# KirillHit/snn_for_object_detection

Hardware: AMD Instinct MI355X
Metric: event-frames/sec (BxT) SODa-3M GEN1 304x240 fwd+bwd (higher is better)
Workload: dtype f32 (16-bit split products)

## Files before the change

### include/snn_hip.h

```cpp
#ifndef SNN_HIP_H
#define SNN_HIP_H

#include <stddef.h>
#include <stdint.h>

#ifdef __cplusplus
extern "C" {
#endif

#define SNN_ABI_VERSION 11

enum {
    SNN_NEURON_NONE = 0,
    SNN_NEURON_LIF = 1,
    SNN_NEURON_LI = 2,
    SNN_NEURON_LI_TANH = 3,
    SNN_NEURON_SLI = 4,
    SNN_NEURON_SYNAPSE = 5
};

enum { SNN_PREC_FP32 = 0, SNN_PREC_BF16X3 = 1, SNN_PREC_BF16X6 = 3, SNN_PREC_FP16X3 = 4, SNN_PREC_BF16X1 = 5,
       SNN_PREC_BF16S = 6 };

enum { SNN_SCAN_WIDE_ADDRESSING = 1,
       SNN_SCAN_LAST_STEP_ONLY = 2,
       SNN_SCAN_BF16_STORAGE = 4,
       SNN_SCAN_SPIKES_FROM_VDEC = 8,
       SNN_SCAN_SUMS_FROM_STATE = 16,
       SNN_SCAN_STATE_LOOKBACK = 32   };

enum { SNN_POOL_AVG = 0, SNN_POOL_MAX = 1, SNN_POOL_SUM = 2 };

enum { SNN_ACT_RELU = 0, SNN_ACT_SILU = 1, SNN_ACT_TANH = 2 };

typedef struct snn_neuron_params {
    float c_mem;
    float c_syn;
    float v_leak;
    float v_th;
    float v_reset;
    float alpha;
    float v_st;
    float tau_sec;
    float tau_dis;
    float dt;
    float sigma;
} snn_neuron_params;

int snn_abi_version(void);
const char* snn_last_error(void);

int snn_nchw_to_nhwc(const float* src, float* dst, int64_t N, int C, int H, int W, void* stream);
int snn_nhwc_to_nchw(const float* src, float* dst, int64_t N, int C, int H, int W, void* stream);
int snn_weight_transpose(const float* w, float* wt, int Cout, int KH, int KW, int Cin, void* stream);
int snn_weight_transpose_batched(const float* flat_w, float* flat_wt, const int64_t* table, int n_layers, void* stream);
int snn_weight_presplit(const float* w, void* out, int64_t n, int precision, void* stream);

int snn_conv2d_wgrad_bn_supported(int64_t N, int H, int W, int Cin, int Ho, int Wo, int Cout, int KH, int KW, int stride,
                                  int pad);
int snn_conv2d_wgrad_bn(const float* x, int64_t ldx, const float* gx, int64_t ldgx, const float* y, int64_t ldy,
                        const float* coef, int T, int frames_per_step, float* dw, int64_t N, int H, int W, int Cin, int Ho,
                        int Wo, int Cout, int KH, int KW, int stride, int pad, int accumulate, float* workspace, int splitk,
                        void* stream);
int snn_conv3x3_s2_dgrad_supported(int64_t N, int H, int W, int Cin, int Ho, int Wo, int Cout);
int snn_conv3x3_s2_dgrad(const float* dy, int64_t lddy, const void* wt_image, float* dx, int64_t lddx, int64_t N, int H, int W,
                         int Cin, int Ho, int Wo, int Cout, const float* addend, int64_t ld_addend, const float* addend2,
                         int64_t ld_addend2, int precision , void* stream);
int snn_conv3x3_halo_bn_supported(int64_t N, int H, int W, int Cin, int Cout, int frames_per_step);
int snn_conv3x3_halo_bn(const float* gx, const float* y, const float* coef, int frames_per_step, float* dy_out,
                        const void* wt_image, float* dx, int64_t lddx, int64_t N, int H, int W, int Cin, int Cout,
                        const float* addend, int64_t ld_addend, const float* addend2, int64_t ld_addend2, void* stream);
int snn_conv3x3_halo_supported(int64_t N, int H, int W, int Cin, int Cout);
int64_t snn_conv3x3_halo_bn_chunks(int frames_per_step, int H, int W);
size_t snn_weight_frag_image_bytes(int O, int I);
int snn_weight_frag_image_batched(const float* flat_src, void* flat_dst, const int64_t* table, int n, int max_threads,
                                  int flip, int precision, void* stream);
int snn_conv3x3_halo(const float* x, int64_t ldx, const void* w_image, float* y, int64_t ldy, int64_t N, int H, int W,
                     int Cin, int Cout, const float* addend, int64_t ld_addend, const float* addend2, int64_t ld_addend2,
                     double* bn_partial, int frames_per_step, int* bn_layout, int precision, void* stream);
size_t snn_conv2d_fwd_bn_partial_size(int64_t N, int frames_per_step, int Ho, int Wo, int Cout);
int snn_conv2d_fwd(const float* x, int64_t ldx, const float* w, const void* w_split, float* y, int64_t ldy,
                   int64_t N, int H, int W, int Cin, int Ho, int Wo, int Cout,
                   int KH, int KW, int stride, int pad, const float* addend, int64_t ld_addend,
                   double* bn_partial, int frames_per_step, int* bn_layout, int precision, void* stream);
int snn_conv2d_dgrad(const float* dy, int64_t lddy, const float* wt, const void* wt_split, float* dx, int64_t lddx,
                     int64_t N, int H, int W, int Cin, int Ho, int Wo, int Cout,
                     int KH, int KW, int stride, int pad, const float* addend, int64_t ld_addend,
                     const float* addend2, int64_t ld_addend2, int precision, void* stream);
int snn_conv2d_wgrad(const float* x, int64_t ldx, const float* dy, int64_t lddy, float* dw,
                     int64_t N, int H, int W, int Cin, int Ho, int Wo, int Cout,
                     int KH, int KW, int stride, int pad, int accumulate,
                     float* workspace, int splitk, int precision, void* stream);
int snn_conv2d_wgrad_splitk(int64_t N, int H, int W, int Cin, int Ho, int Wo, int Cout, int KH, int KW,
                            int stride, int pad, int precision);
int snn_conv2d_wgrad_kernel(int64_t N, int H, int W, int Cin, int Ho, int Wo, int Cout, int KH, int KW, int stride, int pad,
                            int precision);
int snn_conv1x1_spikes_supported(int64_t N, int H, int W, int Cin, int Cout, int64_t ld, int fwd_precision,
                                 int bwd_precision);
int snn_conv1x1_spikes_fwd(const float* vdec, int64_t ld, float v_th, const float* w, float* y, int64_t ldy, int64_t N, int H,
                           int W, int Cin, int Cout, void* stream);
int snn_conv1x1_spikes_wgrad(const float* vdec, int64_t ld, float v_th, const float* dy, int64_t lddy, float* dw, int64_t N,
                             int H, int W, int Cin, int Cout, int accumulate, float* workspace, int splitk, void* stream);

int snn_conv2d_spikes_supported(int64_t N, int H, int W, int Cin, int Ho, int Wo, int Cout, int KH, int KW, int stride,
                                int pad, int64_t ld, int fwd_precision, int bwd_precision);
int snn_conv2d_spikes_fwd(const float* vdec, int64_t ld, float v_th, const float* w, float* y, int64_t ldy, int64_t N, int H,
                          int W, int Cin, int Ho, int Wo, int Cout, int KH, int KW, int stride, int pad, double* bn_partial,
                          int frames_per_step, int* bn_layout, void* stream);
int snn_conv2d_spikes_wgrad(const float* vdec, int64_t ld, float v_th, const float* dy, int64_t lddy, float* dw, int64_t N,
                            int H, int W, int Cin, int Ho, int Wo, int Cout, int KH, int KW, int stride, int pad,
                            int accumulate, float* workspace, int splitk, void* stream);
int snn_conv3x3_halo_spikes(const float* vdec, int64_t ld, float v_th, const void* w_image, float* y, int64_t ldy, int64_t N,
                            int H, int W, int Cin, int Cout, double* bn_partial, int frames_per_step, int* bn_layout,
                            void* stream);

size_t snn_bn_stats_partial_size(int T, int64_t M, int C);
int snn_bn_stats(const float* y, int64_t ldy, int T, int64_t M, int C, double* partial, void* stream);
int snn_bn_stats_finalize(const double* partial, int chunks, int rows_per_chunk, int T, int64_t M, int C,
                          const float* gamma, const float* bias, float eps, float momentum,
                          float* running_mean, float* running_var, int use_running,
                          float* mean, float* invstd, float* alpha, float* beta, void* stream);

int snn_bn_stats_reduce(const double* partial, int chunks, int rows_per_chunk, int T, int64_t M, int C, double* sums,
                        void* stream);
int snn_bn_stats_from_sums(const double* sums, int T, int64_t M_total, int C,
                           const float* gamma, const float* bias, float eps, float momentum,
                           float* running_mean, float* running_var,
                           float* mean, float* invstd, float* alpha, float* beta,
                           double* var_scratch, void* stream);

int snn_affine_neuron_fwd(int neuron, const float* y, int64_t ldy,
                          const float* alpha, const float* beta,
                          const float* v0, const float* i0,
                          float* out, int64_t ldo, const float* addend, int64_t ld_addend,
                          float* vT, float* iT, float* vdec,
                          int T, int64_t M, int C, const snn_neuron_params* p, int flags, void* stream);

size_t snn_affine_neuron_bwd_sums_size(int T, int64_t M, int C);
int snn_affine_neuron_bwd_sums_from_state(int neuron, int T, int64_t M, int C, int64_t ldg, const snn_neuron_params* p,
                                          int flags);
int snn_affine_neuron_bwd(int neuron, const float* g_out, int64_t ldg, const float* state,
                          const float* y, int64_t ldy, const float* g_vT, const float* g_iT,
                          const float* alpha, const float* beta, int apply_scale,
                          float* gx, float* g_v0, float* g_i0, double* sums,
                          int T, int64_t M, int C, const snn_neuron_params* p, int flags, void* stream);

int snn_lif_ckpt_interval(void);
int snn_lif_fwd_ckpt(const float* y, int64_t ldy, const float* alpha, const float* beta,
                     const float* v0, const float* i0, float* out, int64_t ldo,
                     const float* addend, int64_t ld_addend, float* vT, float* iT, float* ckpt,
                     int T, int64_t M, int C, const snn_neuron_params* p, void* stream);
int snn_lif_bwd_ckpt(const float* g_out, int64_t ldg, const float* ckpt, const float* y, int64_t ldy,
                     const float* g_vT, const float* g_iT, const float* alpha, const float* beta, int apply_scale,
                     float* gx, float* g_v0, float* g_i0, double* sums,
                     int T, int64_t M, int C, const snn_neuron_params* p, void* stream);

int snn_bn_bwd_finalize(double* sums, int T, int64_t M, int C,
                        const float* gamma, const float* mean, const float* invstd,
                        float* coefA, float* coefB, float* coefC,
                        float* dgamma, float* dbias, int accumulate, void* stream);
int snn_bn_bwd_finalize_from_state(double* sums, int T, int64_t M, int C,
                                   const float* gamma, const float* bias, const float* mean, const float* invstd,
                                   const float* gx, const float* y, int64_t ldy,
                                   float* coefA, float* coefB, float* coefC,
                                   float* dgamma, float* dbias, int accumulate, void* stream);
int snn_bn_bwd_reduce(const double* sums, int T, int64_t M, int C, double* raw, void* stream);
int snn_bn_bwd_reduce_from_state(const double* sums, int T, int64_t M, int C, const float* gamma, const float* bias,
                                 const float* mean, const float* invstd, const float* gx, const float* y, int64_t ldy,
                                 double* raw, void* stream);
int snn_bn_bwd_coef(const double* raw, const double* raw_local, double* param_sums, int T, int64_t M_total, int C,
                    const float* gamma, const float* mean, const float* invstd,
                    float* coefA, float* coefB, float* coefC,
                    float* dgamma, float* dbias, int accumulate, void* stream);
int snn_bn_bwd_apply(const float* gx, const float* y, int64_t ldy,
                     const float* coefA, const float* coefB, const float* coefC,
                     float* dy, int64_t lddy, int T, int64_t M, int C, int accumulate, void* stream);
int snn_bn_bwd_apply_bf16(const float* gx, const float* y, int64_t ldy, const float* coefA, const float* coefB,
                          const float* coefC, float* dy, int64_t lddy, int T, int64_t M, int C, int accumulate, void* stream);
int snn_bn_stats_bf16(const float* y, int64_t ldy, int T, int64_t M, int C, double* partial, void* stream);

int snn_copy_channels(const float* src, int64_t lds, float* dst, int64_t ldd, int64_t M, int C, void* stream);
int snn_add_channels(const float* src, int64_t lds, float* dst, int64_t ldd, int64_t M, int C, void* stream);
int snn_add(const float* a, int64_t lda, const float* b, int64_t ldb, float* dst, int64_t ldd,
            int64_t M, int C, void* stream);
int snn_copy_channels_bf16(const float* src, int64_t lds, float* dst, int64_t ldd, int64_t M, int C, void* stream);
int snn_add_bf16(const float* a, int64_t lda, const float* b, int64_t ldb, float* dst, int64_t ldd, int64_t M, int C,
                 void* stream);
int snn_convert_bf16(const void* src, void* dst, int64_t n, int to_bf16, void* stream);
int snn_act_fwd(int act, const float* x, float* y, int64_t n, void* stream);
int snn_act_bwd(int act, const float* x, const float* y, const float* gy, float* gx, int64_t n, void* stream);

int snn_small_gemm(const float* A, int64_t lda, int transA, const float* B, int64_t ldb, int transB, float* C,
                  int64_t ldc, int M, int N, int K, int accumulate, float* Ct, int64_t ldct, void* stream);
int snn_small_gemm_batched(const float* base_a, const float* base_b, float* base_c, float* base_ct, const int64_t* table,
                           int n, int max_tiles, void* stream);

int snn_lstm_cell_fwd(const float* gates, const float* c_prev, float* h, float* c, int64_t M, int C, void* stream);
int snn_lstm_cell_bwd(const float* gates, const float* c_prev, const float* c, const float* gh, const float* gc,
                      float* g_gates, float* g_c_prev, int64_t M, int C, void* stream);

int snn_pool_fwd(int kind, const float* x, float* y, int64_t N, int H, int W, int C,
                 int Ho, int Wo, int k, int stride, void* stream);
int snn_pool_bwd(int kind, const float* x, const float* gy, float* gx, int64_t N, int H, int W, int C,
                 int Ho, int Wo, int k, int stride, void* stream);
int snn_upsample_fwd(const float* x, float* y, int64_t N, int H, int W, int C, int scale, void* stream);
int snn_upsample_bwd(const float* gy, float* gx, int64_t N, int H, int W, int C, int scale, void* stream);

int snn_adamax_step(float* param, const float* grad, float* exp_avg, float* exp_inf,
                    int64_t n, float lr, float beta1, float beta2, float eps, int step,
                    float grad_scale, void* stream);

int snn_events_to_frames(const int32_t* t_bin, const int32_t* x, const int32_t* y, const int32_t* p,
                         int64_t n_events, float* frames, int T, int H, int W, void* stream);

int snn_detect_decode(const float* cls_prob, const float* offsets, const float* anchors, int A, int K,
                      float* conf, int* cls, float* boxes, void* stream);
int snn_nms_sorted(const float* boxes, const int* order, const int* seg, int num_classes, float iou_threshold,
                   int* kept, int* nkept, unsigned char* kept_flag, int* kept_rank, void* stream);

size_t snn_roi_workspace_size(int B, int A, int N);
int snn_roi_assign(const float* anchors, const float* labels, int B, int A, int N, float iou_threshold,
                   void* workspace, float* bbox_offset, float* bbox_mask, int64_t* class_labels, void* stream);
size_t snn_det_loss_workspace_size(int64_t rows);
int snn_det_loss_fwd(const float* cls_logits, const float* bbox_preds, const float* bbox_offset, const float* bbox_mask,
                     const int64_t* class_labels, int64_t rows, int K, float loss_ratio, void* workspace, double* stats,
                     float* loss, void* stream);
int snn_det_loss_bwd(const float* cls_logits, const float* bbox_preds, const float* bbox_offset, const float* bbox_mask,
                     const int64_t* class_labels, int64_t rows, int K, float loss_ratio, const double* stats,
                     const float* g_loss, float* g_logits, float* g_bbox, void* stream);

#ifdef __cplusplus
}
#endif
#endif
```

### snn_for_object_detection_amd/_hip.py

```python

import ctypes
import os
from ctypes import POINTER, Structure, c_char_p, c_double, c_float, c_int, c_int32, c_int64, c_size_t, c_void_p

_HERE = os.path.dirname(os.path.abspath(__file__))
LIB_PATH = os.environ.get("SNN_HIP_LIB") or os.path.join(_HERE, "libsnn_hip.so")

NEURON_NONE, NEURON_LIF, NEURON_LI, NEURON_LI_TANH, NEURON_SLI, NEURON_SYNAPSE = 0, 1, 2, 3, 4, 5
POOL_AVG, POOL_MAX, POOL_SUM = 0, 1, 2
ACT_RELU, ACT_SILU, ACT_TANH = 0, 1, 2
ABI_VERSION = 11
PREC_FP32, PREC_BF16X3, PREC_BF16X6, PREC_FP16X3, PREC_BF16X1, PREC_BF16S = 0, 1, 3, 4, 5, 6
SCAN_WIDE_ADDRESSING, SCAN_LAST_STEP_ONLY, SCAN_BF16_STORAGE, SCAN_SPIKES_FROM_VDEC, SCAN_SUMS_FROM_STATE = 1, 2, 4, 8, 16
SCAN_STATE_LOOKBACK = 32


class NeuronParams(Structure):
    _fields_ = [("c_mem", c_float), ("c_syn", c_float), ("v_leak", c_float), ("v_th", c_float),
                ("v_reset", c_float), ("alpha", c_float), ("v_st", c_float), ("tau_sec", c_float),
                ("tau_dis", c_float), ("dt", c_float), ("sigma", c_float)]


_P, _I, _L, _F = c_void_p, c_int, c_int64, c_float

SIGNATURES = {
    "snn_abi_version": (c_int, []),
    "snn_last_error": (c_char_p, []),
    "snn_nchw_to_nhwc": (c_int, [_P, _P, _L, _I, _I, _I, _P]),
    "snn_nhwc_to_nchw": (c_int, [_P, _P, _L, _I, _I, _I, _P]),
    "snn_weight_transpose": (c_int, [_P, _P, _I, _I, _I, _I, _P]),
    "snn_weight_transpose_batched": (c_int, [_P, _P, _P, _I, _P]),
    "snn_detect_decode": (c_int, [_P, _P, _P, _I, _I, _P, _P, _P, _P]),
    "snn_nms_sorted": (c_int, [_P, _P, _P, _I, _F, _P, _P, _P, _P, _P]),
    "snn_conv2d_fwd": (c_int, [_P, _L, _P, _P, _P, _L, _L, _I, _I, _I, _I, _I, _I, _I, _I, _I, _I, _P, _L, _P, _I, _P, _I,
                               _P]),
    "snn_weight_presplit": (c_int, [_P, _P, _L, _I, _P]),
    "snn_conv2d_fwd_bn_partial_size": (c_size_t, [_L, _I, _I, _I, _I]),
    "snn_conv2d_wgrad_bn_supported": (c_int, [_L, _I, _I, _I, _I, _I, _I, _I, _I, _I, _I]),
    "snn_conv2d_wgrad_bn": (c_int, [_P, _L, _P, _L, _P, _L, _P, _I, _I, _P, _L, _I, _I, _I, _I, _I, _I, _I, _I, _I, _I, _I,
                                    _P, _I, _P]),
    "snn_conv3x3_s2_dgrad_supported": (c_int, [_L, _I, _I, _I, _I, _I, _I]),
    "snn_conv3x3_s2_dgrad": (c_int, [_P, _L, _P, _P, _L, _L, _I, _I, _I, _I, _I, _I, _P, _L, _P, _L, _I, _P]),
    "snn_conv3x3_halo_bn_supported": (c_int, [_L, _I, _I, _I, _I, _I]),
    "snn_conv3x3_halo_bn": (c_int, [_P, _P, _P, _I, _P, _P, _P, _L, _L, _I, _I, _I, _I, _P, _L, _P, _L, _P]),
    "snn_conv3x3_halo_supported": (c_int, [_L, _I, _I, _I, _I]),
    "snn_conv3x3_halo_bn_chunks": (c_int64, [_I, _I, _I]),
    "snn_weight_frag_image_bytes": (c_size_t, [_I, _I]),
    "snn_weight_frag_image_batched": (c_int, [_P, _P, _P, _I, _I, _I, _I, _P]),
    "snn_conv3x3_halo": (c_int, [_P, _L, _P, _P, _L, _L, _I, _I, _I, _I, _P, _L, _P, _L, _P, _I, _P, _I, _P]),
    "snn_conv2d_dgrad": (c_int, [_P, _L, _P, _P, _P, _L, _L, _I, _I, _I, _I, _I, _I, _I, _I, _I, _I, _P, _L, _P, _L,
                                 _I, _P]),
    "snn_conv2d_wgrad": (c_int, [_P, _L, _P, _L, _P, _L, _I, _I, _I, _I, _I, _I, _I, _I, _I, _I, _I, _P, _I, _I,
                                 _P]),
    "snn_conv2d_wgrad_splitk": (c_int, [_L, _I, _I, _I, _I, _I, _I, _I, _I, _I, _I, _I]),
    "snn_conv2d_wgrad_kernel": (c_int, [_L, _I, _I, _I, _I, _I, _I, _I, _I, _I, _I, _I]),
    "snn_conv1x1_spikes_supported": (c_int, [_L, _I, _I, _I, _I, _L, _I, _I]),
    "snn_conv1x1_spikes_fwd": (c_int, [_P, _L, _F, _P, _P, _L, _L, _I, _I, _I, _I, _P]),
    "snn_conv1x1_spikes_wgrad": (c_int, [_P, _L, _F, _P, _L, _P, _L, _I, _I, _I, _I, _I, _P, _I, _P]),
    "snn_conv2d_spikes_supported": (c_int, [_L, _I, _I, _I, _I, _I, _I, _I, _I, _I, _I, _L, _I, _I]),
    "snn_conv2d_spikes_fwd": (c_int, [_P, _L, _F, _P, _P, _L, _L, _I, _I, _I, _I, _I, _I, _I, _I, _I, _I, _P, _I, _P, _P]),
    "snn_conv2d_spikes_wgrad": (c_int, [_P, _L, _F, _P, _L, _P, _L, _I, _I, _I, _I, _I, _I, _I, _I, _I, _I, _I, _P, _I, _P]),
    "snn_conv3x3_halo_spikes": (c_int, [_P, _L, _F, _P, _P, _L, _L, _I, _I, _I, _I, _P, _I, _P, _P]),
    "snn_bn_stats_partial_size": (c_size_t, [_I, _L, _I]),
    "snn_bn_stats": (c_int, [_P, _L, _I, _L, _I, _P, _P]),
    "snn_bn_stats_finalize": (c_int, [_P, _I, _I, _I, _L, _I, _P, _P, _F, _F, _P, _P, _I, _P, _P, _P, _P, _P]),
    "snn_bn_stats_reduce": (c_int, [_P, _I, _I, _I, _L, _I, _P, _P]),
    "snn_bn_stats_from_sums": (c_int, [_P, _I, _L, _I, _P, _P, _F, _F, _P, _P, _P, _P, _P, _P, _P, _P]),
    "snn_bn_bwd_reduce": (c_int, [_P, _I, _L, _I, _P, _P]),
    "snn_bn_bwd_coef": (c_int, [_P, _P, _P, _I, _L, _I, _P, _P, _P, _P, _P, _P, _P, _P, _I, _P]),
    "snn_affine_neuron_fwd": (c_int, [_I, _P, _L, _P, _P, _P, _P, _P, _L, _P, _L, _P, _P, _P, _I, _L, _I,
                                      POINTER(NeuronParams), _I, _P]),
    "snn_lif_ckpt_interval": (c_int, []),
    "snn_lif_fwd_ckpt": (c_int, [_P, _L, _P, _P, _P, _P, _P, _L, _P, _L, _P, _P, _P, _I, _L, _I,
                                 POINTER(NeuronParams), _P]),
    "snn_lif_bwd_ckpt": (c_int, [_P, _L, _P, _P, _L, _P, _P, _P, _P, _I, _P, _P, _P, _P, _I, _L, _I,
                                 POINTER(NeuronParams), _P]),
    "snn_affine_neuron_bwd_sums_size": (c_size_t, [_I, _L, _I]),
    "snn_affine_neuron_bwd": (c_int, [_I, _P, _L, _P, _P, _L, _P, _P, _P, _P, _I, _P, _P, _P, _P, _I, _L, _I,
                                      POINTER(NeuronParams), _I, _P]),
    "snn_bn_bwd_finalize": (c_int, [_P, _I, _L, _I, _P, _P, _P, _P, _P, _P, _P, _P, _I, _P]),
    "snn_bn_bwd_finalize_from_state": (c_int, [_P, _I, _L, _I, _P, _P, _P, _P, _P, _P, _L, _P, _P, _P, _P, _P, _I, _P]),
    "snn_bn_bwd_reduce_from_state": (c_int, [_P, _I, _L, _I, _P, _P, _P, _P, _P, _P, _L, _P, _P]),
    "snn_affine_neuron_bwd_sums_from_state": (c_int, [_I, _I, _L, _I, _L, POINTER(NeuronParams), _I]),
    "snn_bn_bwd_apply": (c_int, [_P, _P, _L, _P, _P, _P, _P, _L, _I, _L, _I, _I, _P]),
    "snn_bn_bwd_apply_bf16": (c_int, [_P, _P, _L, _P, _P, _P, _P, _L, _I, _L, _I, _I, _P]),
    "snn_bn_stats_bf16": (c_int, [_P, _L, _I, _L, _I, _P, _P]),
    "snn_copy_channels": (c_int, [_P, _L, _P, _L, _L, _I, _P]),
    "snn_add_channels": (c_int, [_P, _L, _P, _L, _L, _I, _P]),
    "snn_add": (c_int, [_P, _L, _P, _L, _P, _L, _L, _I, _P]),
    "snn_roi_workspace_size": (c_size_t, [_I, _I, _I]),
    "snn_roi_assign": (c_int, [_P, _P, _I, _I, _I, _F, _P, _P, _P, _P, _P]),
    "snn_det_loss_workspace_size": (c_size_t, [_L]),
    "snn_det_loss_fwd": (c_int, [_P, _P, _P, _P, _P, _L, _I, _F, _P, _P, _P, _P]),
    "snn_det_loss_bwd": (c_int, [_P, _P, _P, _P, _P, _L, _I, _F, _P, _P, _P, _P, _P]),
    "snn_small_gemm": (c_int, [_P, _L, _I, _P, _L, _I, _P, _L, _I, _I, _I, _I, _P, _L, _P]),
    "snn_small_gemm_batched": (c_int, [_P, _P, _P, _P, _P, _I, _I, _P]),
    "snn_copy_channels_bf16": (c_int, [_P, _L, _P, _L, _L, _I, _P]),
    "snn_add_bf16": (c_int, [_P, _L, _P, _L, _P, _L, _L, _I, _P]),
    "snn_convert_bf16": (c_int, [_P, _P, _L, _I, _P]),
    "snn_act_fwd": (c_int, [_I, _P, _P, _L, _P]),
    "snn_act_bwd": (c_int, [_I, _P, _P, _P, _P, _L, _P]),
    "snn_lstm_cell_fwd": (c_int, [_P, _P, _P, _P, _L, _I, _P]),
    "snn_lstm_cell_bwd": (c_int, [_P, _P, _P, _P, _P, _P, _P, _L, _I, _P]),
    "snn_pool_fwd": (c_int, [_I, _P, _P, _L, _I, _I, _I, _I, _I, _I, _I, _P]),
    "snn_pool_bwd": (c_int, [_I, _P, _P, _P, _L, _I, _I, _I, _I, _I, _I, _I, _P]),
    "snn_upsample_fwd": (c_int, [_P, _P, _L, _I, _I, _I, _I, _P]),
    "snn_upsample_bwd": (c_int, [_P, _P, _L, _I, _I, _I, _I, _P]),
    "snn_adamax_step": (c_int, [_P, _P, _P, _P, _L, _F, _F, _F, _F, _I, _F, _P]),
    "snn_events_to_frames": (c_int, [_P, _P, _P, _P, _L, _P, _I, _I, _I, _P]),
}

_lib = None


def load():
    global _lib
    if _lib is not None:
        return _lib
    if not os.path.exists(LIB_PATH):
        raise RuntimeError(
            f"{LIB_PATH} not found: the gfx950 HIP extension has not been built "
            "(run `python -m snn_for_object_detection_amd._build`); there is no CPU / eager fallback")
    if not os.environ.get("SNN_HIP_LIB"):
        from . import _build
        if not _build.library_is_current():
            raise RuntimeError(
                f"{LIB_PATH} was not built from the kernel sources as they are now (csrc/*.hip, include/snn_hip.h "
                "changed, or the build stamp is missing): run `python -m snn_for_object_detection_amd._build`")
    lib = ctypes.CDLL(LIB_PATH)
    for name, (res, args) in SIGNATURES.items():
        fn = getattr(lib, name)
        fn.restype, fn.argtypes = res, args
    if lib.snn_abi_version() != ABI_VERSION:
        raise RuntimeError(f"libsnn_hip.so ABI {lib.snn_abi_version()} != binding {ABI_VERSION}: rebuild")
    _lib = lib
    return lib


PROFILER = None


def call(name: str, *args) -> None:
    lib = load()
    if PROFILER is not None:
        token = PROFILER.before(name, args)
        rc = getattr(lib, name)(*args)
        PROFILER.after(token)
    else:
        rc = getattr(lib, name)(*args)
    if rc != 0:
        msg = lib.snn_last_error()
        raise RuntimeError(f"{name} failed (rc={rc}): {msg.decode() if msg else '?'}")


def query(name: str, *args):
    return getattr(load(), name)(*args)
```

### snn_for_object_detection_amd/csrc/conv_halo.hip

```cpp
#include <stdlib.h>
#include <type_traits>
#include "snn_common.h"

namespace {

constexpr int kThreads = 256;
constexpr int HBM_ = 128;
constexpr int HCELLS = 288;
constexpr int HPIECE = HCELLS * 64;
constexpr int NPASS = HCELLS / 32;
static_assert(NPASS == 9, "one halo staging pass per tap");

typedef __bf16 bf16x8 __attribute__((ext_vector_type(8)));
typedef __bf16 bf16x2 __attribute__((ext_vector_type(2)));
typedef _Float16 f16x8 __attribute__((ext_vector_type(8)));
typedef _Float16 f16x2 __attribute__((ext_vector_type(2)));
typedef float f32x2 __attribute__((ext_vector_type(2)));
typedef unsigned u32x2 __attribute__((ext_vector_type(2)));
typedef unsigned u32x4 __attribute__((ext_vector_type(4)));

constexpr float kF16WeightScale = 256.0f;
constexpr float kF16ActScale = 16.0f;
constexpr float kF16Unscale = 1.0f / (kF16WeightScale * kF16ActScale);

struct HaloGeom {
    int64_t ldx, ldy, ld_add, ld_add2;
    int N, H, W, Cin, Cout;
    int PW, PH;
    int G;
    int group_cells;
    int tiles_per_group, tiles, tiles_per_xcd, ntiles_n;
    unsigned magic_pw, magic_ph;
    int out_vec;
    double* bn_partial;
    int OH, OW;
    int bn_T, bn_tc, bn_fps;
    int tiles_x, tiles_img;
    float x_th;
};

__device__ __forceinline__ unsigned udiv_small(unsigned n, unsigned magic) { return __umulhi(n, magic); }

template <bool F16>
__device__ __forceinline__ void split4(const f32x4& v, u32x2& hi, u32x2& lo) {
#pragma unroll
    for (int e = 0; e < 4; e += 2) {
        if constexpr (F16) {
            const float a = v[e] * kF16ActScale, b = v[e + 1] * kF16ActScale;
            const f16x2 ph = __builtin_convertvector(f32x2{a, b}, f16x2);
            const f16x2 pl = __builtin_convertvector(f32x2{a - (float)ph[0], b - (float)ph[1]}, f16x2);
            hi[e >> 1] = __builtin_bit_cast(unsigned, ph);
            lo[e >> 1] = __builtin_bit_cast(unsigned, pl);
        } else {
            f32x2 rest = {v[e], v[e + 1]};
            const bf16x2 ph = __builtin_convertvector(rest, bf16x2);
            const unsigned bits = __builtin_bit_cast(unsigned, ph);
            rest[0] -= __builtin_bit_cast(float, bits << 16);
            rest[1] -= __builtin_bit_cast(float, bits & 0xffff0000u);
            const bf16x2 pl = __builtin_convertvector(rest, bf16x2);
            hi[e >> 1] = bits;
            lo[e >> 1] = __builtin_bit_cast(unsigned, pl);
        }
    }
}

__device__ __forceinline__ double partner8(double v) {
    const u32x2 u = __builtin_bit_cast(u32x2, v);
    const u32x2 o = {(unsigned)__builtin_amdgcn_update_dpp(0, (int)u[0], 0x128, 0xf, 0xf, false),
                     (unsigned)__builtin_amdgcn_update_dpp(0, (int)u[1], 0x128, 0xf, 0xf, false)};
    return __builtin_bit_cast(double, o);
}
__device__ __forceinline__ double partner16(double v) {
    const u32x2 u = __builtin_bit_cast(u32x2, v);
    const u32x2 o = {__builtin_amdgcn_permlane16_swap(u[0], u[0], false, false)[0],
                     __builtin_amdgcn_permlane16_swap(u[1], u[1], false, false)[0]};
    return __builtin_bit_cast(double, o);
}
__device__ __forceinline__ double partner32(double v) {
    const u32x2 u = __builtin_bit_cast(u32x2, v);
    const u32x2 o = {__builtin_amdgcn_permlane32_swap(u[0], u[0], false, false)[0],
                     __builtin_amdgcn_permlane32_swap(u[1], u[1], false, false)[0]};
    return __builtin_bit_cast(double, o);
}

__device__ __forceinline__ int cell_slot_off(int cell, int slot) { return cell * 64 + ((slot ^ ((cell >> 2) & 3)) << 4); }

constexpr int BN_NT = 3;
constexpr int BN_CMAX = 128;

constexpr int RTH = 4, RTW = 32, RPITCH = RTW + 2, RCELLS = (RTH + 2) * RPITCH;

template <int CO, bool F16, int ABL = 0, bool BNAP = false, bool RECT = false, bool SBF = false, bool XSP = false>
__global__ __launch_bounds__(kThreads, 2) void k_conv_halo3(const float* __restrict__ x,
                                                           const unsigned char* __restrict__ wimg,
                                                           float* __restrict__ y, HaloGeom g,
                                                           const float* __restrict__ addend,
                                                           const float* __restrict__ addend2,
                                                           const float* __restrict__ bn_y = nullptr,
                                                           const float* __restrict__ bn_coef = nullptr,
                                                           float* __restrict__ dy_out = nullptr) {
    constexpr int WM = CO == 32 ? 4 : 2, WN = 4 / WM, TM = CO == 32 ? 1 : 2, TN = CO == 32 ? 1 : CO / 64;
    static_assert(CO == 32 || CO == 64 || CO == 128, "channel tile");
    static_assert(!BNAP || CO >= 64, "the BatchNorm-apply variant covers the 64 / 128-channel tiles");
    constexpr int BTILE = (CO / 32) * 4096;
    constexpr int NDMA = (CO / 32) * 4 / 4;
    constexpr int ES = SBF ? 2 : 4;
    static_assert(!SBF || (!F16 && !BNAP && ABL == 0), "bf16 storage: bf16 MFMA, plain variant");
    static_assert(!XSP || (F16 && !BNAP && !SBF && ABL == 0), "spikes from potentials: the forward arithmetic, plain variant");
    constexpr int CF_BYTES = BNAP ? 3 * BN_NT * BN_CMAX * 4 : 0;
    constexpr int HC = RECT ? (RCELLS + 31) / 32 * 32 : HCELLS;
    constexpr int HP = HC * 64;
    constexpr int RED_BYTES = (F16 || SBF) ? 4 * (CO == 128 ? 64 : 32) * 16 : 0;
    __shared__ __attribute__((aligned(16))) unsigned char smem[2 * HP + 2 * BTILE + CF_BYTES + RED_BYTES];
    unsigned char* Aimg = smem;
    unsigned char* Bimg = smem + 2 * HP;
    [[maybe_unused]] float* Cf = reinterpret_cast<float*>(smem + 2 * HP + 2 * BTILE);

    const int tid = threadIdx.x, lane = tid & 63;
    const int wave = __builtin_amdgcn_readfirstlane(tid >> 6);
    const int wm = wave / WN, wn = wave % WN;
    const int r = lane & 31, h = lane >> 5;

    const int bq = blockIdx.x >> 3;
    const int tile = (blockIdx.x & 7) * g.tiles_per_xcd + bq / g.ntiles_n;
    if (tile >= g.tiles) return;
    const int n0c = (bq % g.ntiles_n) * CO;
    int grp, kt, c0 = 0, x0 = 0, y0 = 0, n0, nb;
    [[maybe_unused]] int ty = 0, tx = 0;
    if constexpr (RECT) {
        n0 = tile / g.tiles_img;
        const int rem = tile - n0 * g.tiles_img;
        ty = rem / g.tiles_x;
        tx = rem - ty * g.tiles_x;
        grp = n0 / g.G;
        kt = (n0 - grp * g.G) * g.tiles_img + rem;
        nb = n0;
    } else {
        grp = tile / g.tiles_per_group;
        kt = tile - grp * g.tiles_per_group;
        c0 = kt * HBM_;
        const int R0g = c0 / g.PW;
        x0 = c0 - R0g * g.PW;
        const int ng = R0g / g.PH;
        y0 = R0g - ng * g.PH;
        n0 = grp * g.G + ng;
        nb = n0 > 0 ? n0 - 1 : 0;
    }
    const int pitch = RECT ? RPITCH : g.PW;

    const int quad = tid & 7;
    const int64_t ipix = (int64_t)g.H * g.W;
    const int64_t xbytes = ((((int64_t)g.N - nb) * ipix - 1) * g.ldx + g.Cin) * ES;
    __amdgpu_buffer_rsrc_t rs_x = __builtin_amdgcn_make_buffer_rsrc(
        reinterpret_cast<char*>(const_cast<float*>(x)) + (int64_t)nb * ipix * g.ldx * ES, 0,
        xbytes > 0x7fffffffLL ? 0x7fffffff : (int)xbytes, 0x00020000);
    [[maybe_unused]] __amdgpu_buffer_rsrc_t rs_y = rs_x, rs_dy = rs_x;
    [[maybe_unused]] const int t_lo = BNAP ? nb / g.bn_fps : 0;
    [[maybe_unused]] int cofs[NPASS];
    [[maybe_unused]] unsigned imask = 0;
    [[maybe_unused]] unsigned vmask = 0;
    if constexpr (BNAP) {
        rs_y = __builtin_amdgcn_make_buffer_rsrc(const_cast<float*>(bn_y + (int64_t)nb * ipix * g.ldx), 0,
                                                 xbytes > 0x7fffffffLL ? 0x7fffffff : (int)xbytes, 0x00020000);
        rs_dy = __builtin_amdgcn_make_buffer_rsrc(dy_out + (int64_t)nb * ipix * g.ldx, 0,
                                                  xbytes > 0x7fffffffLL ? 0x7fffffff : (int)xbytes, 0x00020000);
        for (int idx = tid; idx < 3 * BN_NT * g.Cin; idx += kThreads) {
            const int pl = idx / (BN_NT * g.Cin), rem = idx - pl * BN_NT * g.Cin;
            const int k = rem / g.Cin, c = rem - k * g.Cin;
            const int t = t_lo + k < g.bn_T ? t_lo + k : g.bn_T - 1;
            Cf[idx] = bn_coef[(int64_t)pl * g.bn_tc + (int64_t)t * g.Cin + c];
        }
    }
    unsigned voff[NPASS];
    int awr[NPASS];
#pragma unroll
    for (int p = 0; p < NPASS; ++p) {
        const int cell = p * 32 + (tid >> 3);
        int xx, yy, n;
        bool ok;
        if constexpr (RECT) {
            const int rr = cell / RPITCH, cc = cell - rr * RPITCH;
            yy = ty * RTH - 1 + rr;
            xx = tx * RTW - 1 + cc;
            n = n0;
            ok = cell < RCELLS && yy >= 0 && yy < g.H && xx >= 0 && xx < g.W;
        } else {
            const unsigned u = (unsigned)(x0 + cell + g.PW - 1);
            const unsigned dR = udiv_small(u, g.magic_pw);
            xx = (int)(u - dR * g.PW);
            const unsigned v = (unsigned)(y0 + (int)dR + g.PH - 2);
            const unsigned dn = udiv_small(v, g.magic_ph);
            yy = (int)(v - dn * g.PH);
            n = n0 - 1 + (int)dn;
            ok = n >= 0 && n < g.N && xx < g.W && yy < g.H;
        }
        const int64_t pix = (int64_t)(n - nb) * ipix + (int64_t)yy * g.W + xx;
        voff[p] = ok ? (unsigned)((pix * g.ldx + quad * 4) * ES) : 0x80000000u;
        awr[p] = cell_slot_off(cell, quad >> 1) + (quad & 1) * 8;
        if constexpr (BNAP) {
            int ts = ok ? n / g.bn_fps - t_lo : 0;
            ts = ts < BN_NT ? ts : BN_NT - 1;
            cofs[p] = ts * g.Cin + quad * 4;
            bool mine;
            if constexpr (RECT) {
                const int rr = cell / RPITCH, cc = cell - rr * RPITCH;
                mine = rr >= 1 && rr <= RTH && cc >= 1 && cc <= RTW;
            } else {
                const int m = cell - (g.PW + 1);
                mine = m >= 0 && m < HBM_ && m < g.group_cells - c0;
            }
            imask |= (ok && mine) ? 1u << p : 0u;
            vmask |= ok ? 1u << p : 0u;
        }
    }

    int cellbase[TM];
#pragma unroll
    for (int i = 0; i < TM; ++i)
        cellbase[i] = RECT ? (wm * TM + i + 1) * RPITCH + 1 + r : g.PW + 1 + (wm * TM + i) * 32 + r;
    const int nchunks = g.Cin >> 5;
    const int co_tiles = g.Cout >> 5;
    const unsigned char* wsrc = wimg + (int64_t)(n0c >> 5) * 4096 + lane * 16;
    const unsigned lds_b = (unsigned)(size_t)(__attribute__((address_space(3))) unsigned char*)Bimg;
    auto dma_b = [&](int kk, int buf) {
        if constexpr (SBF)
            if (wave & 1) return;
        const int chunk = kk / 9, tap = kk - chunk * 9;
        const unsigned char* src = wsrc + ((int64_t)(tap * nchunks + chunk) * co_tiles) * 4096 + wave * 1024;
        const unsigned dst = lds_b + buf * BTILE + wave * 1024;
#pragma unroll
        for (int q = 0; q < NDMA; ++q) {
            unsigned keep;
            asm volatile("s_mov_b32 %0, m0\n\ts_mov_b32 m0, %2\n\ts_nop 0\n\tglobal_load_lds_dwordx4 %1, off\n\ts_mov_b32 m0, %0"
                         : "=&s"(keep)
                         : "v"(src + q * 4096), "s"(__builtin_amdgcn_readfirstlane(dst + q * 4096))
                         : "memory");
        }
    };

    using PReg = typename std::conditional<SBF, u32x2, f32x4>::type;
    PReg pf[NPASS];
    auto store_halo = [&]() {
#pragma unroll
        for (int p = 0; p < NPASS; ++p) {
            if constexpr (RECT)
                if (p * 32 >= HC) continue;
            if constexpr (SBF) {
                *reinterpret_cast<u32x2*>(Aimg + awr[p]) = pf[p];
            } else if constexpr (XSP) {
                const u32x2 hi = {(pf[p][0] > g.x_th ? 0x4C00u : 0u) | (pf[p][1] > g.x_th ? 0x4C000000u : 0u),
                                  (pf[p][2] > g.x_th ? 0x4C00u : 0u) | (pf[p][3] > g.x_th ? 0x4C000000u : 0u)};
                *reinterpret_cast<u32x2*>(Aimg + awr[p]) = hi;
            } else {
                u32x2 hi, lo;
                split4<F16>(pf[p], hi, lo);
                *reinterpret_cast<u32x2*>(Aimg + awr[p]) = hi;
                *reinterpret_cast<u32x2*>(Aimg + HP + awr[p]) = lo;
            }
        }
    };
    auto load_pass = [&](int off) -> PReg {
        if constexpr (SBF) return __builtin_bit_cast(u32x2, __builtin_amdgcn_raw_buffer_load_b64(rs_x, off, 0, 0));
        else return __builtin_bit_cast(f32x4, __builtin_amdgcn_raw_buffer_load_b128(rs_x, off, 0, 0));
    };

    [[maybe_unused]] f32x4 pfy[2];
    [[maybe_unused]] auto bn_combine = [&](f32x4& gxv, const f32x4& yv, int p, int chan_floats, bool live) {
        const int planes = BN_NT * g.Cin;
        const float* cf = Cf + cofs[p] + chan_floats;
        const f32x4 ca = *reinterpret_cast<const f32x4*>(cf), cb = *reinterpret_cast<const f32x4*>(cf + planes),
                    cc = *reinterpret_cast<const f32x4*>(cf + 2 * planes);
#pragma unroll
        for (int e = 0; e < 4; ++e) gxv[e] = ca[e] * gxv[e] + cb[e] * yv[e] + cc[e];
        if (!((vmask >> p) & 1u)) gxv = f32x4{0.f, 0.f, 0.f, 0.f};
        const unsigned so = (live && ((imask >> p) & 1u)) ? voff[p] + (unsigned)chan_floats * 4u : 0x80000000u;
        __builtin_amdgcn_raw_buffer_store_b128(__builtin_bit_cast(u32x4, gxv), rs_dy, (int)so, 0, 0);
    };

    f32x16 acc[TM][TN];
#pragma unroll
    for (int i = 0; i < TM; ++i)
#pragma unroll
        for (int j = 0; j < TN; ++j)
#pragma unroll
            for (int e = 0; e < 16; ++e) acc[i][j][e] = 0.f;

    auto kstep = [&](int tapoff, const unsigned char* Bb) {
#pragma unroll
        for (int ks = 0; ks < 2; ++ks) {
            bf16x8 ah[TM], al[TM], bh[TN], bl[TN];
#pragma unroll
            for (int i = 0; i < TM; ++i) {
                const int off = cell_slot_off(cellbase[i] + tapoff, 2 * ks + h);
                if constexpr (ABL & 16) {
                    if (i == 0 && ks == 0) ah[0] = *reinterpret_cast<const bf16x8*>(Aimg + off);
                    ah[i] = ah[0];
                    al[i] = ah[0];
                    continue;
                }
                ah[i] = *reinterpret_cast<const bf16x8*>(Aimg + off);
                if constexpr (!SBF && !XSP) al[i] = *reinterpret_cast<const bf16x8*>(Aimg + HP + off);
            }
#pragma unroll
            for (int j = 0; j < TN; ++j) {
                const int off = (wn * TN + j) * 4096 + ks * 2048 + lane * 16;
                bh[j] = *reinterpret_cast<const bf16x8*>(Bb + off);
                if constexpr (!SBF) bl[j] = *reinterpret_cast<const bf16x8*>(Bb + off + 1024);
            }
#pragma unroll
            for (int i = 0; i < TM; ++i)
#pragma unroll
                for (int j = 0; j < TN; ++j) {
                    if constexpr (SBF) {
                        acc[i][j] = __builtin_amdgcn_mfma_f32_32x32x16_bf16(ah[i], bh[j], acc[i][j], 0, 0, 0);
                    } else if constexpr (XSP) {
                        const f16x8 xah = __builtin_bit_cast(f16x8, ah[i]);
                        const f16x8 xbh = __builtin_bit_cast(f16x8, bh[j]), xbl = __builtin_bit_cast(f16x8, bl[j]);
                        acc[i][j] = __builtin_amdgcn_mfma_f32_32x32x16_f16(xah, xbl, acc[i][j], 0, 0, 0);
                        acc[i][j] = __builtin_amdgcn_mfma_f32_32x32x16_f16(xah, xbh, acc[i][j], 0, 0, 0);
                    } else if constexpr (F16) {
                        const f16x8 xah = __builtin_bit_cast(f16x8, ah[i]), xal = __builtin_bit_cast(f16x8, al[i]);
                        const f16x8 xbh = __builtin_bit_cast(f16x8, bh[j]), xbl = __builtin_bit_cast(f16x8, bl[j]);
                        acc[i][j] = __builtin_amdgcn_mfma_f32_32x32x16_f16(xal, xbh, acc[i][j], 0, 0, 0);
                        acc[i][j] = __builtin_amdgcn_mfma_f32_32x32x16_f16(xah, xbl, acc[i][j], 0, 0, 0);
                        acc[i][j] = __builtin_amdgcn_mfma_f32_32x32x16_f16(xah, xbh, acc[i][j], 0, 0, 0);
                    } else {
                        acc[i][j] = __builtin_amdgcn_mfma_f32_32x32x16_bf16(al[i], bh[j], acc[i][j], 0, 0, 0);
                        acc[i][j] = __builtin_amdgcn_mfma_f32_32x32x16_bf16(ah[i], bl[j], acc[i][j], 0, 0, 0);
                        acc[i][j] = __builtin_amdgcn_mfma_f32_32x32x16_bf16(ah[i], bh[j], acc[i][j], 0, 0, 0);
                    }
                }
        }
    };

    dma_b(0, 0);
#pragma unroll
    for (int p = 0; p < NPASS; ++p) pf[p] = load_pass((int)voff[p]);
    if constexpr (BNAP) {
        f32x4 py[NPASS];
#pragma unroll
        for (int p = 0; p < NPASS; ++p)
            py[p] = __builtin_bit_cast(f32x4, __builtin_amdgcn_raw_buffer_load_b128(rs_y, (int)voff[p], 0, 0));
        __syncthreads();
#pragma unroll
        for (int p = 0; p < NPASS; ++p) bn_combine(pf[p], py[p], p, 0, true);
    }
    store_halo();
    asm volatile("s_waitcnt vmcnt(0) lgkmcnt(0)\n\ts_barrier" ::: "memory");

    const int nk = nchunks * 9;
#pragma unroll 1
    for (int chunk = 0; chunk < nchunks; ++chunk) {
        const bool more = chunk + 1 < nchunks;
        const int cbytes = (chunk + 1) * 32 * ES;
#pragma unroll
        for (int tap = 0; tap < 9; ++tap) {
            const int kk = chunk * 9 + tap;
            const int cur = kk & 1;
            if constexpr (!(ABL & 1))
                if (kk + 1 < nk) dma_b(kk + 1, cur ^ 1);
            __builtin_amdgcn_sched_barrier(0);
            if constexpr (!(ABL & 4)) {
                if (BNAP || more) pf[tap] = load_pass(more ? (int)(voff[tap] + (unsigned)cbytes) : (int)0x80000000u);
            }
            if constexpr (BNAP)
                pfy[tap & 1] = __builtin_bit_cast(f32x4, __builtin_amdgcn_raw_buffer_load_b128(
                                                              rs_y, more ? (int)(voff[tap] + (unsigned)cbytes) : (int)0x80000000u, 0, 0));
            __builtin_amdgcn_sched_barrier(0);
            const int kh = tap / 3, kw = tap - 3 * kh;
            kstep((kh - 1) * pitch + (kw - 1), Bimg + cur * BTILE);
            if constexpr (BNAP) {
                const int pp = tap >= 1 ? tap - 1 : 0;
                __builtin_amdgcn_sched_barrier(0);
                if (tap >= 1) bn_combine(pf[pp], pfy[pp & 1], pp, more ? (chunk + 1) * 32 : 0, more);
                __builtin_amdgcn_sched_barrier(0);
                asm volatile("s_waitcnt vmcnt(0) lgkmcnt(0)\n\ts_barrier" ::: "memory");
            } else if constexpr (ABL & 2) asm volatile("" ::: "memory");
            else if constexpr (ABL & 4) asm volatile("s_waitcnt vmcnt(0) lgkmcnt(0)\n\ts_barrier" ::: "memory");
            else asm volatile("s_waitcnt vmcnt(0) lgkmcnt(0)\n\ts_barrier" ::: "memory");
        }
        if (more) {
            if constexpr (BNAP) bn_combine(pf[8], pfy[0], 8, (chunk + 1) * 32, true);
            store_halo();
            asm volatile("s_waitcnt lgkmcnt(0)\n\ts_barrier" ::: "memory");
        }
    }

    constexpr int EW = TN * 32 + 4;
    constexpr int LPR = TN * 8;
    constexpr int RPP = 64 / LPR;
    float* stage = reinterpret_cast<float*>(smem) + wave * 32 * EW;
    const bool ovec = g.out_vec != 0;
    const int lrow = lane / LPR, c4 = (lane % LPR) * 4;
    const int nch = n0c + wn * TN * 32 + c4;
    const int cells_left = g.group_cells - c0;
    double ssum[4] = {0.0, 0.0, 0.0, 0.0}, qsum[4] = {0.0, 0.0, 0.0, 0.0};
    const bool stats = (F16 || SBF) && g.bn_partial != nullptr;
    auto cell_pixel = [&](int m, int64_t& pix) -> bool {
        int xx, yy, n;
        bool ok;
        if constexpr (RECT) {
            yy = ty * RTH + (m >> 5);
            xx = tx * RTW + (m & 31);
            n = n0;
            ok = yy < g.H && xx < g.W && nch < g.Cout;
        } else {
            const unsigned u = (unsigned)(x0 + m);
            const unsigned dR = udiv_small(u, g.magic_pw);
            xx = (int)(u - dR * g.PW);
            const unsigned v = (unsigned)(y0 + (int)dR);
            const unsigned dn = udiv_small(v, g.magic_ph);
            yy = (int)(v - dn * g.PH);
            n = n0 + (int)dn;
            ok = m < cells_left && xx < g.W && yy < g.H && n < g.N && nch < g.Cout;
        }
        pix = ((int64_t)n * g.H + yy) * g.W + xx;
        return ok;
    };
    typedef SnnStore<SBF> St;
    constexpr int NPS = 32 / RPP;
    const bool prefetch_add = ovec && (addend != nullptr || addend2 != nullptr) && !(ABL & 8);
#pragma unroll
    for (int i = 0; i < TM; ++i) {
        f32x4 pa1[NPS], pa2[NPS];
        int64_t ppix[NPS];
        unsigned okmask = 0;
        if (prefetch_add) {
#pragma unroll
            for (int pass = 0; pass < NPS; ++pass) {
                const bool ok = cell_pixel((wm * TM + i) * 32 + pass * RPP + lrow, ppix[pass]);
                okmask |= ok ? 1u << pass : 0u;
                const int64_t pc = ok ? ppix[pass] : 0;
                const int nc = ok ? nch : 0;
                const f32x4 zero = {0.f, 0.f, 0.f, 0.f};
                pa1[pass] = addend ? St::ld4_last(addend, pc * g.ld_add + nc) : zero;
                pa2[pass] = addend2 ? St::ld4_last(addend2, pc * g.ld_add2 + nc) : zero;
            }
        }
#pragma unroll
        for (int j = 0; j < TN; ++j)
#pragma unroll
            for (int e = 0; e < 16; ++e)
                stage[((e & 3) + 8 * (e >> 2) + 4 * h) * EW + j * 32 + r] = F16 ? acc[i][j][e] * kF16Unscale : acc[i][j][e];
        asm volatile("s_waitcnt lgkmcnt(0)" ::: "memory");
        if (prefetch_add) {
#pragma unroll
            for (int pass = 0; pass < NPS; ++pass) {
                f32x4 val = *reinterpret_cast<const f32x4*>(&stage[(pass * RPP + lrow) * EW + c4]);
                if (addend) val += pa1[pass];
                if (addend2) val += pa2[pass];
                if ((okmask >> pass) & 1u) St::st4(y, ppix[pass] * g.ldy + nch, val);
            }
            asm volatile("s_waitcnt lgkmcnt(0)" ::: "memory");
            continue;
        }
#pragma unroll
        for (int pass = 0; pass < NPS; ++pass) {
            const int row = pass * RPP + lrow;
            int64_t pix;
            const bool ok = cell_pixel((wm * TM + i) * 32 + row, pix);
            f32x4 val = *reinterpret_cast<const f32x4*>(&stage[row * EW + c4]);
            if (!ok) continue;
            if constexpr (ABL & 8) {
                asm volatile("" :: "v"(val[0]), "v"(val[1]), "v"(val[2]), "v"(val[3]));
                continue;
            }
            if (ovec) {
                if (addend) val += St::ld4_last(addend, pix * g.ld_add + nch);
                if (addend2) val += St::ld4_last(addend2, pix * g.ld_add2 + nch);
                St::st4(y, pix * g.ldy + nch, val);
            } else {
#pragma unroll
                for (int q = 0; q < 4; ++q) {
                    float o = val[q];
                    if (addend) o += St::ld1(addend, pix * g.ld_add + nch + q);
                    if (addend2) o += St::ld1(addend2, pix * g.ld_add2 + nch + q);
                    St::st1(y, pix * g.ldy + nch + q, o);
                }
            }
            if (stats) {
#pragma unroll
                for (int q = 0; q < 4; ++q) {
                    const double d = (double)val[q];
                    ssum[q] += d;
                    qsum[q] = fma(d, d, qsum[q]);
                }
            }
        }
        asm volatile("s_waitcnt lgkmcnt(0)" ::: "memory");
    }
    if (stats) {
#pragma unroll
        for (int q = 0; q < 4; ++q) {
            if constexpr (LPR <= 8) {
                ssum[q] += partner8(ssum[q]);
                qsum[q] += partner8(qsum[q]);
            }
            ssum[q] += partner16(ssum[q]);
            qsum[q] += partner16(qsum[q]);
            ssum[q] += partner32(ssum[q]);
            qsum[q] += partner32(qsum[q]);
        }
        double* red = reinterpret_cast<double*>(smem + 2 * HP + 2 * BTILE + CF_BYTES);
        if (lane >= 48 && lane < 48 + LPR) {
#pragma unroll
            for (int q = 0; q < 4; ++q) {
                red[((wave * LPR + lane - 48) * 4 + q) * 2 + 0] = ssum[q];
                red[((wave * LPR + lane - 48) * 4 + q) * 2 + 1] = qsum[q];
            }
        }
        __syncthreads();
        if (tid < CO) {
            const int wn_ = tid / (TN * 32), cc = tid % (TN * 32);
            double s = 0.0, q2 = 0.0;
#pragma unroll
            for (int wm_ = 0; wm_ < WM; ++wm_) {
                const double* src = red + (((wm_ * WN + wn_) * LPR * 4) + cc) * 2;
                s += src[0];
                q2 += src[1];
            }
            if (n0c + tid < g.Cout) {
                double* dstp = g.bn_partial + snn_bn_partial_index(grp, kt, n0c + tid, g.tiles_per_group, g.Cout);
                dstp[0] = s;
                dstp[1] = q2;
            }
        }
    }
}

constexpr int SPITCH = RTW + 1, SCELLS = (RTH + 1) * SPITCH;
template <bool SBF = false, bool RECT = false>
__global__ __launch_bounds__(kThreads, 2) void k_conv_s2dgrad3(const float* __restrict__ x,
                                                              const unsigned char* __restrict__ wimg,
                                                              float* __restrict__ y,
                                                              HaloGeom g, const float* __restrict__ addend,
                                                              const float* __restrict__ addend2) {
    constexpr int CO = 64, TN = 2;
    constexpr int ES = SBF ? 2 : 4;
    constexpr int BTILE = (CO / 32) * 4096;
    constexpr int NDMA = (CO / 32) * 4 / 4;
    __shared__ __attribute__((aligned(16))) unsigned char smem[2 * HPIECE + 2 * BTILE];
    unsigned char* Aimg = smem;
    unsigned char* Bimg = smem + 2 * HPIECE;

    const int tid = threadIdx.x, lane = tid & 63;
    const int wave = __builtin_amdgcn_readfirstlane(tid >> 6);
    const int r = lane & 31, h = lane >> 5;

    const int bq = blockIdx.x >> 3;
    const int tile = (blockIdx.x & 7) * g.tiles_per_xcd + bq / g.ntiles_n;
    if (tile >= g.tiles) return;
    const int n0c = (bq % g.ntiles_n) * CO;
    int c0 = 0, x0 = 0, y0 = 0, n0;
    [[maybe_unused]] int ty = 0, tx = 0;
    if constexpr (RECT) {
        n0 = tile / g.tiles_img;
        const int rem = tile - n0 * g.tiles_img;
        ty = rem / g.tiles_x;
        tx = rem - ty * g.tiles_x;
    } else {
        c0 = tile * HBM_;
        const int R0g = c0 / g.PW;
        x0 = c0 - R0g * g.PW;
        n0 = R0g / g.PH;
        y0 = R0g - n0 * g.PH;
    }
    const int nb = n0;
    const int pitch = RECT ? SPITCH : g.PW;

    const int quad = tid & 7;
    const int64_t ipix = (int64_t)g.H * g.W;
    const int64_t xbytes = ((((int64_t)g.N - nb) * ipix - 1) * g.ldx + g.Cin) * ES;
    __amdgpu_buffer_rsrc_t rs_x = __builtin_amdgcn_make_buffer_rsrc(
        reinterpret_cast<char*>(const_cast<float*>(x)) + (int64_t)nb * ipix * g.ldx * ES, 0,
        xbytes > 0x7fffffffLL ? 0x7fffffff : (int)xbytes, 0x00020000);
    unsigned voff[NPASS];
    int awr[NPASS];
#pragma unroll
    for (int p = 0; p < NPASS; ++p) {
        const int cell = p * 32 + (tid >> 3);
        int xx, yy, n;
        bool ok;
        if constexpr (RECT) {
            const int rr = cell / SPITCH, cc = cell - rr * SPITCH;
            yy = ty * RTH + rr;
            xx = tx * RTW + cc;
            n = n0;
            ok = cell < SCELLS && xx < g.W && yy < g.H;
        } else {
            const unsigned u = (unsigned)(x0 + cell);
            const unsigned dR = udiv_small(u, g.magic_pw);
            xx = (int)(u - dR * g.PW);
            const unsigned v = (unsigned)(y0 + (int)dR);
            const unsigned dn = udiv_small(v, g.magic_ph);
            yy = (int)(v - dn * g.PH);
            n = n0 + (int)dn;
            ok = n < g.N && xx < g.W && yy < g.H;
        }
        const int64_t pix = (int64_t)(n - nb) * ipix + (int64_t)yy * g.W + xx;
        voff[p] = ok ? (unsigned)((pix * g.ldx + quad * 4) * ES) : 0x80000000u;
        awr[p] = cell_slot_off(cell, quad >> 1) + (quad & 1) * 8;
    }
    const int cellbase = RECT ? wave * SPITCH + r : wave * 32 + r;
    const int nchunks = g.Cin >> 5;
    const int co_tiles = g.Cout >> 5;
    const unsigned char* wsrc = wimg + (int64_t)(n0c >> 5) * 4096 + lane * 16;
    const unsigned lds_b = (unsigned)(size_t)(__attribute__((address_space(3))) unsigned char*)Bimg;
    auto dma_b = [&](int kk, int buf) {
        if constexpr (SBF)
            if (wave & 1) return;
        const int chunk = kk / 9, tap = kk - chunk * 9;
        const unsigned char* src = wsrc + ((int64_t)((8 - tap) * nchunks + chunk) * co_tiles) * 4096 + wave * 1024;
        const unsigned dst = lds_b + buf * BTILE + wave * 1024;
#pragma unroll
        for (int q = 0; q < NDMA; ++q) {
            unsigned keep;
            asm volatile("s_mov_b32 %0, m0\n\ts_mov_b32 m0, %2\n\ts_nop 0\n\tglobal_load_lds_dwordx4 %1, off\n\ts_mov_b32 m0, %0"
                         : "=&s"(keep)
                         : "v"(src + q * 4096), "s"(__builtin_amdgcn_readfirstlane(dst + q * 4096))
                         : "memory");
        }
    };
    using PReg = typename std::conditional<SBF, u32x2, f32x4>::type;
    PReg pf[NPASS];
    auto store_halo = [&]() {
#pragma unroll
        for (int p = 0; p < NPASS; ++p) {
            if constexpr (SBF) {
                *reinterpret_cast<u32x2*>(Aimg + awr[p]) = pf[p];
            } else {
                u32x2 hi, lo;
                split4<false>(pf[p], hi, lo);
                *reinterpret_cast<u32x2*>(Aimg + awr[p]) = hi;
                *reinterpret_cast<u32x2*>(Aimg + HPIECE + awr[p]) = lo;
            }
        }
    };
    auto load_pass = [&](int off) -> PReg {
        if constexpr (SBF) return __builtin_bit_cast(u32x2, __builtin_amdgcn_raw_buffer_load_b64(rs_x, off, 0, 0));
        else return __builtin_bit_cast(f32x4, __builtin_amdgcn_raw_buffer_load_b128(rs_x, off, 0, 0));
    };
    f32x16 acc[4][TN];
#pragma unroll
    for (int c = 0; c < 4; ++c)
#pragma unroll
        for (int j = 0; j < TN; ++j)
#pragma unroll
            for (int e = 0; e < 16; ++e) acc[c][j][e] = 0.f;

    auto kstep = [&](int tapoff, const unsigned char* Bb, f32x16 (&a)[TN]) {
#pragma unroll
        for (int ks = 0; ks < 2; ++ks) {
            const int off = cell_slot_off(cellbase + tapoff, 2 * ks + h);
            const bf16x8 ah = *reinterpret_cast<const bf16x8*>(Aimg + off);
            bf16x8 al = ah;
            if constexpr (!SBF) al = *reinterpret_cast<const bf16x8*>(Aimg + HPIECE + off);
#pragma unroll
            for (int j = 0; j < TN; ++j) {
                const int boff = j * 4096 + ks * 2048 + lane * 16;
                const bf16x8 bh = *reinterpret_cast<const bf16x8*>(Bb + boff);
                if constexpr (!SBF) {
                    const bf16x8 bl = *reinterpret_cast<const bf16x8*>(Bb + boff + 1024);
                    a[j] = __builtin_amdgcn_mfma_f32_32x32x16_bf16(al, bh, a[j], 0, 0, 0);
                    a[j] = __builtin_amdgcn_mfma_f32_32x32x16_bf16(ah, bl, a[j], 0, 0, 0);
                }
                a[j] = __builtin_amdgcn_mfma_f32_32x32x16_bf16(ah, bh, a[j], 0, 0, 0);
            }
        }
    };

    dma_b(0, 0);
#pragma unroll
    for (int p = 0; p < NPASS; ++p) pf[p] = load_pass((int)voff[p]);
    store_halo();
    asm volatile("s_waitcnt vmcnt(0) lgkmcnt(0)\n\ts_barrier" ::: "memory");

    const int nk = nchunks * 9;
#pragma unroll 1
    for (int chunk = 0; chunk < nchunks; ++chunk) {
        const bool more = chunk + 1 < nchunks;
        const int cbytes = (chunk + 1) * 32 * ES;
#pragma unroll
        for (int tap = 0; tap < 9; ++tap) {
            const int kk = chunk * 9 + tap;
            const int cur = kk & 1;
            if (kk + 1 < nk) dma_b(kk + 1, cur ^ 1);
            __builtin_amdgcn_sched_barrier(0);
            if (more) pf[tap] = load_pass((int)(voff[tap] + (unsigned)cbytes));
            __builtin_amdgcn_sched_barrier(0);
            const int kh = tap / 3, kw = tap - 3 * kh;
            const int ph = kh == 1 ? 0 : 1, pw = kw == 1 ? 0 : 1;
            const int dh = kh == 0 ? 1 : 0, dw = kw == 0 ? 1 : 0;
            kstep(dh * pitch + dw, Bimg + cur * BTILE, acc[2 * ph + pw]);
            asm volatile("s_waitcnt vmcnt(0) lgkmcnt(0)\n\ts_barrier" ::: "memory");
        }
        if (more) {
            store_halo();
            asm volatile("s_waitcnt lgkmcnt(0)\n\ts_barrier" ::: "memory");
        }
    }

    constexpr int EW = TN * 32 + 4, LPR = TN * 8, RPP = 64 / LPR;
    float* stage = reinterpret_cast<float*>(smem) + wave * 32 * EW;
    const bool ovec = g.out_vec != 0;
    const int lrow = lane / LPR, c4 = (lane % LPR) * 4;
    const int nch = n0c + c4;
    const int cells_left = g.group_cells - c0;
#pragma unroll
    for (int cls = 0; cls < 4; ++cls) {
        const int ph = cls >> 1, pw = cls & 1;
#pragma unroll
        for (int j = 0; j < TN; ++j)
#pragma unroll
            for (int e = 0; e < 16; ++e)
                stage[((e & 3) + 8 * (e >> 2) + 4 * h) * EW + j * 32 + r] = acc[cls][j][e];
        asm volatile("s_waitcnt lgkmcnt(0)" ::: "memory");
#pragma unroll
        for (int pass = 0; pass < 32 / RPP; ++pass) {
            const int row = pass * RPP + lrow;
            const int m = wave * 32 + row;
            int aa, bb, n;
            bool inside;
            if constexpr (RECT) {
                aa = ty * RTH + wave;
                bb = tx * RTW + row;
                n = n0;
                inside = true;
            } else {
                const unsigned u = (unsigned)(x0 + m);
                const unsigned dR = udiv_small(u, g.magic_pw);
                bb = (int)(u - dR * g.PW);
                const unsigned v = (unsigned)(y0 + (int)dR);
                const unsigned dn = udiv_small(v, g.magic_ph);
                aa = (int)(v - dn * g.PH);
                n = n0 + (int)dn;
                inside = m < cells_left && n < g.N;
            }
            const int hi = 2 * aa + ph, wi = 2 * bb + pw;
            const bool ok = inside && bb < g.W && aa < g.H && hi < g.OH && wi < g.OW && nch < g.Cout;
            f32x4 val = *reinterpret_cast<const f32x4*>(&stage[row * EW + c4]);
            if (!ok) continue;
            const int64_t pix = ((int64_t)n * g.OH + hi) * g.OW + wi;
            typedef SnnStore<SBF> St;
            if (ovec) {
                if (addend) val += St::ld4_last(addend, pix * g.ld_add + nch);
                if (addend2) val += St::ld4_last(addend2, pix * g.ld_add2 + nch);
                St::st4(y, pix * g.ldy + nch, val);
            } else {
#pragma unroll
                for (int q = 0; q < 4; ++q) {
                    float o = val[q];
                    if (addend) o += St::ld1(addend, pix * g.ld_add + nch + q);
                    if (addend2) o += St::ld1(addend2, pix * g.ld_add2 + nch + q);
                    St::st1(y, pix * g.ldy + nch + q, o);
                }
            }
        }
        asm volatile("s_waitcnt lgkmcnt(0)" ::: "memory");
    }
}

template <bool F16>
__global__ void k_weight_frag_image(const float* __restrict__ flat_src, unsigned char* __restrict__ flat_dst,
                                    const int64_t* __restrict__ table, int flip) {
    const int64_t* row = table + (int64_t)blockIdx.y * 4;
    const float* src = flat_src + row[0];
    unsigned char* dst = flat_dst + row[1];
    const int O = (int)row[2], I = (int)row[3];
    const int ot_n = O >> 5, ic_n = I >> 5;
    const int64_t total = (int64_t)9 * ic_n * ot_n * 2 * 64;
    for (int64_t idx = (int64_t)blockIdx.x * blockDim.x + threadIdx.x; idx < total; idx += (int64_t)gridDim.x * blockDim.x) {
        const int lane = (int)(idx & 63);
        const int ks = (int)((idx >> 6) & 1);
        int64_t rest = idx >> 7;
        const int ot = (int)(rest % ot_n); rest /= ot_n;
        const int ic = (int)(rest % ic_n);
        const int tap = (int)(rest / ic_n);
        const int r = lane & 31, h = lane >> 5;
        const int st = flip ? 8 - tap : tap;
        const float* p = src + ((int64_t)(ot * 32 + r) * 9 + st) * I + ic * 32 + ks * 16 + h * 8;
        const f32x4 v0 = *reinterpret_cast<const f32x4*>(p), v1 = *reinterpret_cast<const f32x4*>(p + 4);
        u32x4 hi, lo;
#pragma unroll
        for (int e = 0; e < 8; e += 2) {
            const float a0 = e < 4 ? v0[e] : v1[e - 4], a1 = e < 4 ? v0[e + 1] : v1[e - 3];
            if (F16) {
                const float a = a0 * kF16WeightScale, b = a1 * kF16WeightScale;
                const f16x2 ph = __builtin_convertvector(f32x2{a, b}, f16x2);
                const f16x2 pl = __builtin_convertvector(f32x2{a - (float)ph[0], b - (float)ph[1]}, f16x2);
                hi[e >> 1] = __builtin_bit_cast(unsigned, ph);
                lo[e >> 1] = __builtin_bit_cast(unsigned, pl);
            } else {
                f32x2 rr = {a0, a1};
                const bf16x2 ph = __builtin_convertvector(rr, bf16x2);
                const unsigned bits = __builtin_bit_cast(unsigned, ph);
                rr[0] -= __builtin_bit_cast(float, bits << 16);
                rr[1] -= __builtin_bit_cast(float, bits & 0xffff0000u);
                const bf16x2 pl = __builtin_convertvector(rr, bf16x2);
                hi[e >> 1] = bits;
                lo[e >> 1] = __builtin_bit_cast(unsigned, pl);
            }
        }
        unsigned char* o = dst + ((((int64_t)(tap * ic_n + ic) * ot_n + ot) * 2 + ks) * 2) * 1024 + lane * 16;
        *reinterpret_cast<u32x4*>(o) = hi;
        *reinterpret_cast<u32x4*>(o + 1024) = lo;
    }
}

static unsigned magic_u32(int d) { return (unsigned)((0x100000000ULL + (unsigned)d - 1) / (unsigned)d); }
static bool aligned16(const void* p) { return (reinterpret_cast<uintptr_t>(p) & 15u) == 0; }
static bool aligned8(const void* p) { return (reinterpret_cast<uintptr_t>(p) & 7u) == 0; }
static bool out_aligned(const void* p, bool bf16) { return bf16 ? aligned8(p) : aligned16(p); }

static int halo_mode(int64_t N, int H, int W, int Cin, int Cout) {
    if (N <= 0 || H <= 0 || W <= 0) return 0;
    if (Cin % 32 != 0 || Cin < 32 || (Cout % 64 != 0 && Cout != 32)) return 0;
    if (Cout == 32 && snn_tuning_env("SNN_HALO_NO_CO32")) return 0;
    if (W + 1 <= 79) {
        if (N * (int64_t)(H + 1) * (W + 1) >= 0x7fffffffLL) return 0;
        return 1;
    }
    const int64_t tiles = N * snn_ceil_div(H, RTH) * snn_ceil_div(W, RTW);
    return tiles < 0x7fffffffLL ? 2 : 0;
}
static bool halo_shape_ok(int64_t N, int H, int W, int Cin, int Cout) { return halo_mode(N, H, W, Cin, Cout) != 0; }

static bool s2dgrad_rect(int Wo) { return 128 + (Wo + 1) + 2 > HCELLS; }
static bool s2dgrad_shape_ok(int64_t N, int H, int W, int Cin, int Ho, int Wo, int Cout) {
    if (N <= 0 || H <= 0 || W <= 0) return false;
    if (Ho != (H - 1) / 2 + 1 || Wo != (W - 1) / 2 + 1) return false;
    if (Cout % 32 != 0 || Cout < 32 || Cin % 64 != 0) return false;
    if (s2dgrad_rect(Wo)) return N * snn_ceil_div(Ho, RTH) * snn_ceil_div(Wo, RTW) < 0x7fffffffLL;
    if (N * (int64_t)(Ho + 1) * (Wo + 1) >= 0x7fffffffLL) return false;
    return true;
}
}

extern "C" int snn_conv3x3_s2_dgrad_supported(int64_t N, int H, int W, int Cin, int Ho, int Wo, int Cout) {
    return s2dgrad_shape_ok(N, H, W, Cin, Ho, Wo, Cout) ? 1 : 0;
}

extern "C" int snn_conv3x3_s2_dgrad(const float* dy, int64_t lddy, const void* wt_image, float* dx, int64_t lddx, int64_t N,
                                    int H, int W, int Cin, int Ho, int Wo, int Cout, const float* addend, int64_t ld_addend,
                                    const float* addend2, int64_t ld_addend2, int precision, void* stream) {
    SNN_REQUIRE(dy && wt_image && dx, "snn_conv3x3_s2_dgrad: null pointer");
    SNN_REQUIRE(precision == SNN_PREC_BF16X3 || precision == SNN_PREC_BF16S,
                "snn_conv3x3_s2_dgrad: precision must be SNN_PREC_BF16X3 or SNN_PREC_BF16S (got %d)", precision);
    const bool sbf = precision == SNN_PREC_BF16S;
    SNN_REQUIRE(s2dgrad_shape_ok(N, H, W, Cin, Ho, Wo, Cout),
                "snn_conv3x3_s2_dgrad: shape not covered (N %lld, %dx%d -> %dx%d, %d -> %d channels; ask "
                "snn_conv3x3_s2_dgrad_supported)", (long long)N, H, W, Ho, Wo, Cin, Cout);
    SNN_REQUIRE(lddy >= Cout && lddx >= Cin && lddy % 4 == 0, "snn_conv3x3_s2_dgrad: bad pixel strides (%lld, %lld)",
                (long long)lddy, (long long)lddx);
    SNN_REQUIRE((sbf ? aligned8(dy) : aligned16(dy)) && aligned16(wt_image),
                "snn_conv3x3_s2_dgrad: dy (16 bytes; 8 for bf16) and the weight image (16) must be aligned");
    SNN_REQUIRE(!addend || ld_addend >= Cin, "snn_conv3x3_s2_dgrad: addend pixel stride smaller than channel count");
    SNN_REQUIRE(!addend2 || ld_addend2 >= Cin, "snn_conv3x3_s2_dgrad: addend2 pixel stride smaller than channel count");
    HaloGeom g;
    g.ldx = lddy; g.ldy = lddx; g.ld_add = ld_addend; g.ld_add2 = ld_addend2;
    g.N = (int)N; g.H = Ho; g.W = Wo;
    g.Cin = Cout;
    g.Cout = Cin;
    g.OH = H; g.OW = W;
    g.PW = Wo + 1; g.PH = Ho + 1;
    g.G = (int)N;
    const bool rect = s2dgrad_rect(Wo);
    g.tiles_x = (int)snn_ceil_div(Wo, RTW);
    g.tiles_img = g.tiles_x * (int)snn_ceil_div(Ho, RTH);
    if (rect) {
        g.group_cells = 0;
        g.tiles_per_group = g.tiles_img;
        g.tiles = (int)(N * g.tiles_img);
        SNN_REQUIRE((int64_t)Ho * Wo * lddy * 4 < 0x7fffffffLL, "snn_conv3x3_s2_dgrad: a dy image must span less than 2 GiB");
    } else {
        SNN_REQUIRE((int64_t)4 * Ho * Wo * lddy * 4 < 0x7fffffffLL, "snn_conv3x3_s2_dgrad: four dy images must span less than 2 GiB");
        const int64_t cells = N * (int64_t)g.PH * g.PW;
        g.group_cells = (int)cells;
        g.tiles_per_group = (int)snn_ceil_div(cells, HBM_);
        g.tiles = g.tiles_per_group;
    }
    g.ntiles_n = Cin / 64;
    SNN_REQUIRE((int64_t)g.tiles * g.ntiles_n + 8 < 0x7fffffffLL, "snn_conv3x3_s2_dgrad: grid too large");
    g.tiles_per_xcd = (int)snn_ceil_div(g.tiles, 8);
    g.magic_pw = magic_u32(g.PW); g.magic_ph = magic_u32(g.PH);
    g.out_vec = (lddx % 4 == 0) && out_aligned(dx, sbf) && (!addend || (ld_addend % 4 == 0 && out_aligned(addend, sbf))) &&
                (!addend2 || (ld_addend2 % 4 == 0 && out_aligned(addend2, sbf)));
    g.bn_partial = nullptr;
    g.x_th = 0.0f;
    g.bn_T = g.bn_tc = 0; g.bn_fps = 1;
    dim3 grid((unsigned)((int64_t)g.tiles_per_xcd * 8 * g.ntiles_n));
    const unsigned char* wi = static_cast<const unsigned char*>(wt_image);
    if (sbf && rect)
        hipLaunchKernelGGL((k_conv_s2dgrad3<true, true>), grid, dim3(kThreads), 0, (hipStream_t)stream, dy, wi, dx, g, addend, addend2);
    else if (sbf)
        hipLaunchKernelGGL((k_conv_s2dgrad3<true, false>), grid, dim3(kThreads), 0, (hipStream_t)stream, dy, wi, dx, g, addend, addend2);
    else if (rect)
        hipLaunchKernelGGL((k_conv_s2dgrad3<false, true>), grid, dim3(kThreads), 0, (hipStream_t)stream, dy, wi, dx, g, addend, addend2);
    else
        hipLaunchKernelGGL((k_conv_s2dgrad3<false, false>), grid, dim3(kThreads), 0, (hipStream_t)stream, dy, wi, dx, g, addend, addend2);
    SNN_CHECK_LAUNCH("snn_conv3x3_s2_dgrad");
    return 0;
}

extern "C" int snn_conv3x3_halo_supported(int64_t N, int H, int W, int Cin, int Cout) {
    return halo_shape_ok(N, H, W, Cin, Cout) ? 1 : 0;
}

extern "C" int64_t snn_conv3x3_halo_bn_chunks(int frames_per_step, int H, int W) {
    if (W + 1 <= 79) return snn_ceil_div((int64_t)frames_per_step * (H + 1) * (W + 1), HBM_);
    return (int64_t)frames_per_step * snn_ceil_div(H, RTH) * snn_ceil_div(W, RTW);
}

extern "C" size_t snn_weight_frag_image_bytes(int O, int I) { return (size_t)9 * O * I * 4; }

extern "C" int snn_weight_frag_image_batched(const float* flat_src, void* flat_dst, const int64_t* table, int n,
                                             int max_groups, int flip, int precision, void* stream) {
    SNN_REQUIRE(flat_src && flat_dst && table && n > 0 && max_groups > 0, "snn_weight_frag_image_batched: bad arguments");
    SNN_REQUIRE(precision == SNN_PREC_FP16X3 || precision == SNN_PREC_BF16X3,
                "snn_weight_frag_image: precision must be SNN_PREC_FP16X3 (forward) or SNN_PREC_BF16X3 (data gradient)");
    SNN_REQUIRE(aligned16(flat_src) && aligned16(flat_dst), "snn_weight_frag_image: buffers must be 16-byte aligned");
    int64_t bx = snn_ceil_div(max_groups, kThreads);
    if (bx > 64) bx = 64;
    dim3 grid((unsigned)bx, (unsigned)n);
    if (precision == SNN_PREC_FP16X3)
        hipLaunchKernelGGL(k_weight_frag_image<true>, grid, dim3(kThreads), 0, (hipStream_t)stream, flat_src,
                           static_cast<unsigned char*>(flat_dst), table, flip);
    else
        hipLaunchKernelGGL(k_weight_frag_image<false>, grid, dim3(kThreads), 0, (hipStream_t)stream, flat_src,
                           static_cast<unsigned char*>(flat_dst), table, flip);
    SNN_CHECK_LAUNCH("snn_weight_frag_image_batched");
    return 0;
}

extern "C" int snn_conv3x3_halo_bn_supported(int64_t N, int H, int W, int Cin, int Cout, int frames_per_step) {
    if (halo_mode(N, H, W, Cin, Cout) != 1 || Cin > BN_CMAX || frames_per_step <= 0 || N % frames_per_step != 0) return 0;
    if (Cout != 64 && Cout != 128) return 0;
    const int64_t images = HCELLS / ((int64_t)(H + 1) * (W + 1)) + 2;
    return ((images + frames_per_step - 1) / frames_per_step + 1 <= BN_NT) ? 1 : 0;
}

extern "C" int snn_conv3x3_halo_bn(const float* gx, const float* y, const float* coef, int frames_per_step, float* dy_out,
                                   const void* wt_image, float* dx, int64_t lddx, int64_t N, int H, int W, int Cin,
                                   int Cout, const float* addend, int64_t ld_addend, const float* addend2,
                                   int64_t ld_addend2, void* stream) {
    SNN_REQUIRE(gx && y && coef && dy_out && wt_image && dx, "snn_conv3x3_halo_bn: null pointer");
    SNN_REQUIRE(snn_conv3x3_halo_bn_supported(N, H, W, Cin, Cout, frames_per_step),
                "snn_conv3x3_halo_bn: shape not covered (N %lld, %dx%d, %d -> %d channels, %d frames per step; ask "
                "snn_conv3x3_halo_bn_supported)", (long long)N, H, W, Cin, Cout, frames_per_step);
    SNN_REQUIRE(lddx >= Cout, "snn_conv3x3_halo_bn: dx pixel stride smaller than channel count");
    SNN_REQUIRE(aligned16(gx) && aligned16(y) && aligned16(dy_out) && aligned16(wt_image) && aligned16(coef),
                "snn_conv3x3_halo_bn: operands must be 16-byte aligned");
    SNN_REQUIRE(!addend || ld_addend >= Cout, "snn_conv3x3_halo_bn: addend pixel stride smaller than channel count");
    SNN_REQUIRE(!addend2 || ld_addend2 >= Cout, "snn_conv3x3_halo_bn: addend2 pixel stride smaller than channel count");
    SNN_REQUIRE((int64_t)4 * H * W * Cin * 4 < 0x7fffffffLL, "snn_conv3x3_halo_bn: four images must span less than 2 GiB");
    HaloGeom g;
    g.ldx = Cin; g.ldy = lddx; g.ld_add = ld_addend; g.ld_add2 = ld_addend2;
    g.N = (int)N; g.H = H; g.W = W; g.Cin = Cin; g.Cout = Cout;
    g.PW = W + 1; g.PH = H + 1;
    g.G = (int)N;
    const int64_t group_cells = (int64_t)g.G * g.PH * g.PW;
    g.group_cells = (int)group_cells;
    g.tiles_per_group = (int)snn_ceil_div(group_cells, HBM_);
    g.tiles = g.tiles_per_group;
    const int co_tile = Cout % 128 == 0 ? 128 : 64;
    g.ntiles_n = Cout / co_tile;
    SNN_REQUIRE(g.ntiles_n == 1, "snn_conv3x3_halo_bn: %d output channels need more than one channel tile", Cout);
    g.tiles_per_xcd = (int)snn_ceil_div(g.tiles, 8);
    g.magic_pw = magic_u32(g.PW); g.magic_ph = magic_u32(g.PH);
    g.out_vec = (lddx % 4 == 0) && aligned16(dx) && (!addend || (ld_addend % 4 == 0 && aligned16(addend))) &&
                (!addend2 || (ld_addend2 % 4 == 0 && aligned16(addend2)));
    g.bn_partial = nullptr;
    g.x_th = 0.0f;
    g.OH = H; g.OW = W;
    g.bn_fps = frames_per_step; g.bn_T = (int)(N / frames_per_step); g.bn_tc = g.bn_T * Cin;
    g.tiles_x = g.tiles_img = 0;
    dim3 grid((unsigned)((int64_t)g.tiles_per_xcd * 8));
    const unsigned char* wi = static_cast<const unsigned char*>(wt_image);
    if (co_tile == 128)
        hipLaunchKernelGGL((k_conv_halo3<128, false, 0, true>), grid, dim3(kThreads), 0, (hipStream_t)stream, gx, wi, dx, g,
                           addend, addend2, y, coef, dy_out);
    else
        hipLaunchKernelGGL((k_conv_halo3<64, false, 0, true>), grid, dim3(kThreads), 0, (hipStream_t)stream, gx, wi, dx, g,
                           addend, addend2, y, coef, dy_out);
    SNN_CHECK_LAUNCH("snn_conv3x3_halo_bn");
    return 0;
}

static int conv3x3_halo_impl(const float* x, int64_t ldx, const void* w_image, float* y, int64_t ldy, int64_t N, int H,
                             int W, int Cin, int Cout, const float* addend, int64_t ld_addend, const float* addend2,
                             int64_t ld_addend2, double* bn_partial, int frames_per_step, int* bn_layout,
                             int precision, void* stream, bool xsp, float x_th) {
    SNN_REQUIRE(x && w_image && y, "snn_conv3x3_halo: null pointer");
    SNN_REQUIRE(precision == SNN_PREC_FP16X3 || precision == SNN_PREC_BF16X3 || precision == SNN_PREC_BF16S,
                "snn_conv3x3_halo: precision must be SNN_PREC_FP16X3, SNN_PREC_BF16X3 or SNN_PREC_BF16S (got %d)", precision);
    const bool sbf = precision == SNN_PREC_BF16S;
    SNN_REQUIRE(halo_shape_ok(N, H, W, Cin, Cout),
                "snn_conv3x3_halo: shape not covered (N %lld, %dx%d, %d -> %d channels; ask snn_conv3x3_halo_supported)",
                (long long)N, H, W, Cin, Cout);
    SNN_REQUIRE(ldx >= Cin && ldy >= Cout && ldx % 4 == 0, "snn_conv3x3_halo: bad pixel strides (%lld, %lld)",
                (long long)ldx, (long long)ldy);
    SNN_REQUIRE((sbf ? aligned8(x) : aligned16(x)) && aligned16(w_image),
                "snn_conv3x3_halo: x (16 bytes; 8 for bf16) and the weight image (16) must be aligned");
    SNN_REQUIRE(!addend || ld_addend >= Cout, "snn_conv3x3_halo: addend pixel stride smaller than channel count");
    SNN_REQUIRE(!addend2 || ld_addend2 >= Cout, "snn_conv3x3_halo: addend2 pixel stride smaller than channel count");
    SNN_REQUIRE(!bn_partial || ((precision == SNN_PREC_FP16X3 || sbf) && bn_layout && frames_per_step > 0 &&
                                N % frames_per_step == 0 && !addend && !addend2),
                "snn_conv3x3_halo: statistics need the forward arithmetic, bn_layout, no addend and a frames_per_step "
                "that divides N (%lld frames, %d per step)", (long long)N, frames_per_step);
    SNN_REQUIRE((int64_t)4 * H * W * ldx * 4 < 0x7fffffffLL, "snn_conv3x3_halo: four images must span less than 2 GiB");
    if (bn_layout) bn_layout[0] = bn_layout[1] = 0;
    HaloGeom g;
    g.ldx = ldx; g.ldy = ldy; g.ld_add = ld_addend; g.ld_add2 = ld_addend2;
    g.N = (int)N; g.H = H; g.W = W; g.Cin = Cin; g.Cout = Cout;
    const bool rect = halo_mode(N, H, W, Cin, Cout) == 2;
    g.PW = W + 1; g.PH = H + 1;
    g.G = bn_partial ? frames_per_step : (int)N;
    g.tiles_x = (int)snn_ceil_div(W, RTW);
    g.tiles_img = g.tiles_x * (int)snn_ceil_div(H, RTH);
    int64_t tiles;
    if (rect) {
        g.group_cells = 0;
        g.tiles_per_group = g.G * g.tiles_img;
        tiles = N * (int64_t)g.tiles_img;
        SNN_REQUIRE((int64_t)H * W * ldx * 4 < 0x7fffffffLL, "snn_conv3x3_halo: an image must span less than 2 GiB");
    } else {
        const int64_t group_cells = (int64_t)g.G * g.PH * g.PW;
        g.group_cells = (int)group_cells;
        g.tiles_per_group = (int)snn_ceil_div(group_cells, HBM_);
        tiles = (int64_t)(N / g.G) * g.tiles_per_group;
    }
    const int co_tile = Cout % 128 == 0 ? 128 : (Cout % 64 == 0 ? 64 : 32);
    g.ntiles_n = Cout / co_tile;
    SNN_REQUIRE(tiles * g.ntiles_n + 8 < 0x7fffffffLL, "snn_conv3x3_halo: grid too large");
    g.tiles = (int)tiles;
    g.tiles_per_xcd = (int)snn_ceil_div(tiles, 8);
    g.magic_pw = magic_u32(g.PW); g.magic_ph = magic_u32(g.PH);
    g.out_vec = (ldy % 4 == 0) && out_aligned(y, sbf) && (!addend || (ld_addend % 4 == 0 && out_aligned(addend, sbf))) &&
                (!addend2 || (ld_addend2 % 4 == 0 && out_aligned(addend2, sbf)));
    g.bn_partial = bn_partial;
    g.OH = H; g.OW = W;
    g.bn_T = g.bn_tc = 0; g.bn_fps = 1;
    g.x_th = x_th;
    if (bn_partial) bn_layout[0] = g.tiles_per_group;
    dim3 grid((unsigned)((int64_t)g.tiles_per_xcd * 8 * g.ntiles_n));
    const unsigned char* wi = static_cast<const unsigned char*>(w_image);
    const bool f16 = precision == SNN_PREC_FP16X3;
#define SNN_HALO_LAUNCH(CO_, F16_)                                                                                   \
    do {                                                                                                              \
        if (rect)                                                                                                     \
            hipLaunchKernelGGL((k_conv_halo3<CO_, F16_, 0, false, true>), grid, dim3(kThreads), 0, (hipStream_t)stream, x, wi, \
                               y, g, addend, addend2, nullptr, nullptr, nullptr);                                     \
        else                                                                                                          \
            hipLaunchKernelGGL((k_conv_halo3<CO_, F16_>), grid, dim3(kThreads), 0, (hipStream_t)stream, x, wi, y, g, addend, \
                               addend2, nullptr, nullptr, nullptr);                                                   \
    } while (0)
#ifdef SNN_TUNING
    if (const char* e = snn_tuning_env("SNN_HALO_ABL")) {
        const int abl = atoi(e);
#define SNN_HALO_ABL_LAUNCH(A_) \
        if (abl == A_) { \
            if (co_tile == 128) hipLaunchKernelGGL((k_conv_halo3<128, true, A_>), grid, dim3(kThreads), 0, (hipStream_t)stream, x, wi, y, g, addend, addend2); \
            else hipLaunchKernelGGL((k_conv_halo3<64, true, A_>), grid, dim3(kThreads), 0, (hipStream_t)stream, x, wi, y, g, addend, addend2); \
            SNN_CHECK_LAUNCH("snn_conv3x3_halo"); return 0; }
        SNN_HALO_ABL_LAUNCH(1) SNN_HALO_ABL_LAUNCH(2) SNN_HALO_ABL_LAUNCH(4) SNN_HALO_ABL_LAUNCH(8) SNN_HALO_ABL_LAUNCH(16)
        SNN_HALO_ABL_LAUNCH(3) SNN_HALO_ABL_LAUNCH(7) SNN_HALO_ABL_LAUNCH(15) SNN_HALO_ABL_LAUNCH(31)
#undef SNN_HALO_ABL_LAUNCH
    }
#endif
    if (xsp) {
#define SNN_HALO_LAUNCH_X(CO_)                                                                                       \
    do {                                                                                                              \
        if (rect)                                                                                                     \
            hipLaunchKernelGGL((k_conv_halo3<CO_, true, 0, false, true, false, true>), grid, dim3(kThreads), 0,          \
                               (hipStream_t)stream, x, wi, y, g, addend, addend2, nullptr, nullptr, nullptr);          \
        else                                                                                                          \
            hipLaunchKernelGGL((k_conv_halo3<CO_, true, 0, false, false, false, true>), grid, dim3(kThreads), 0,         \
                               (hipStream_t)stream, x, wi, y, g, addend, addend2, nullptr, nullptr, nullptr);          \
    } while (0)
        if (co_tile == 128) SNN_HALO_LAUNCH_X(128);
        else if (co_tile == 64) SNN_HALO_LAUNCH_X(64);
        else SNN_HALO_LAUNCH_X(32);
#undef SNN_HALO_LAUNCH_X
        SNN_CHECK_LAUNCH("snn_conv3x3_halo_spikes");
        return 0;
    }
    if (sbf) {
#define SNN_HALO_LAUNCH_S(CO_)                                                                                       \
    do {                                                                                                              \
        if (rect)                                                                                                     \
            hipLaunchKernelGGL((k_conv_halo3<CO_, false, 0, false, true, true>), grid, dim3(kThreads), 0, (hipStream_t)stream, x, \
                               wi, y, g, addend, addend2, nullptr, nullptr, nullptr);                                 \
        else                                                                                                          \
            hipLaunchKernelGGL((k_conv_halo3<CO_, false, 0, false, false, true>), grid, dim3(kThreads), 0, (hipStream_t)stream, \
                               x, wi, y, g, addend, addend2, nullptr, nullptr, nullptr);                              \
    } while (0)
        if (co_tile == 128) SNN_HALO_LAUNCH_S(128);
        else if (co_tile == 64) SNN_HALO_LAUNCH_S(64);
        else SNN_HALO_LAUNCH_S(32);
#undef SNN_HALO_LAUNCH_S
        SNN_CHECK_LAUNCH("snn_conv3x3_halo");
        return 0;
    }
    if (co_tile == 128) {
        if (f16) SNN_HALO_LAUNCH(128, true); else SNN_HALO_LAUNCH(128, false);
    } else if (co_tile == 64) {
        if (f16) SNN_HALO_LAUNCH(64, true); else SNN_HALO_LAUNCH(64, false);
    } else {
        if (f16) SNN_HALO_LAUNCH(32, true); else SNN_HALO_LAUNCH(32, false);
    }
#undef SNN_HALO_LAUNCH
    SNN_CHECK_LAUNCH("snn_conv3x3_halo");
    return 0;
}

extern "C" int snn_conv3x3_halo(const float* x, int64_t ldx, const void* w_image, float* y, int64_t ldy, int64_t N, int H,
                                int W, int Cin, int Cout, const float* addend, int64_t ld_addend, const float* addend2,
                                int64_t ld_addend2, double* bn_partial, int frames_per_step, int* bn_layout,
                                int precision, void* stream) {
    return conv3x3_halo_impl(x, ldx, w_image, y, ldy, N, H, W, Cin, Cout, addend, ld_addend, addend2, ld_addend2, bn_partial,
                             frames_per_step, bn_layout, precision, stream, false, 0.0f);
}

extern "C" int snn_conv3x3_halo_spikes(const float* vdec, int64_t ld, float v_th, const void* w_image, float* y, int64_t ldy,
                                       int64_t N, int H, int W, int Cin, int Cout, double* bn_partial, int frames_per_step,
                                       int* bn_layout, void* stream) {
    SNN_REQUIRE(v_th >= 0.0f, "snn_conv3x3_halo_spikes: a negative threshold would turn padding into spikes");
    return conv3x3_halo_impl(vdec, ld, w_image, y, ldy, N, H, W, Cin, Cout, nullptr, 0, nullptr, 0, bn_partial,
                             frames_per_step, bn_layout, SNN_PREC_FP16X3, stream, true, v_th);
}
```

Baseline: 7303.

## Add 256-cell halo tile for fp16x3 conv3x3 and eight-wave s2 dgrad

Adds a BIG variant of the halo conv kernel that covers twice as many output cells per block (256-cell strip or 8-row rect) for 32/64-channel fp16x3 forward. It reuses LDS regions for the reduction and keeps BatchNorm partials at the original slot granularity. The halo prefetch is restructured to load all passes at tap 0 rather than one pass per tap. The stride-2 dgrad kernel now defaults to eight waves with the channel tile split across wave pairs. The aim is better weight-tile reuse and more latency hiding, at the cost of higher register and LDS pressure and fewer blocks.

New measurement: 7395, median of 6. 1.3% higher.

```diff
diff --git a/include/snn_hip.h b/include/snn_hip.h
--- a/include/snn_hip.h
+++ b/include/snn_hip.h
@@ -71,6 +71,7 @@
                         const void* wt_image, float* dx, int64_t lddx, int64_t N, int H, int W, int Cin, int Cout,
                         const float* addend, int64_t ld_addend, const float* addend2, int64_t ld_addend2, void* stream);
 int snn_conv3x3_halo_supported(int64_t N, int H, int W, int Cin, int Cout);
+int snn_conv3x3_halo_kernel(int64_t N, int H, int W, int Cin, int Cout, int precision);
 int64_t snn_conv3x3_halo_bn_chunks(int frames_per_step, int H, int W);
 size_t snn_weight_frag_image_bytes(int O, int I);
 int snn_weight_frag_image_batched(const float* flat_src, void* flat_dst, const int64_t* table, int n, int max_threads,
diff --git a/snn_for_object_detection_amd/_hip.py b/snn_for_object_detection_amd/_hip.py
--- a/snn_for_object_detection_amd/_hip.py
+++ b/snn_for_object_detection_amd/_hip.py
@@ -44,6 +44,7 @@
     "snn_conv3x3_halo_bn_supported": (c_int, [_L, _I, _I, _I, _I, _I]),
     "snn_conv3x3_halo_bn": (c_int, [_P, _P, _P, _I, _P, _P, _P, _L, _L, _I, _I, _I, _I, _P, _L, _P, _L, _P]),
     "snn_conv3x3_halo_supported": (c_int, [_L, _I, _I, _I, _I]),
+    "snn_conv3x3_halo_kernel": (c_int, [_L, _I, _I, _I, _I, _I]),
     "snn_conv3x3_halo_bn_chunks": (c_int64, [_I, _I, _I]),
     "snn_weight_frag_image_bytes": (c_size_t, [_I, _I]),
     "snn_weight_frag_image_batched": (c_int, [_P, _P, _P, _I, _I, _I, _I, _P]),
diff --git a/snn_for_object_detection_amd/csrc/conv_halo.hip b/snn_for_object_detection_amd/csrc/conv_halo.hip
--- a/snn_for_object_detection_amd/csrc/conv_halo.hip
+++ b/snn_for_object_detection_amd/csrc/conv_halo.hip
@@ -7,7 +7,6 @@
 constexpr int kThreads = 256;
 constexpr int HBM_ = 128;
 constexpr int HCELLS = 288;
-constexpr int HPIECE = HCELLS * 64;
 constexpr int NPASS = HCELLS / 32;
 static_assert(NPASS == 9, "one halo staging pass per tap");
 
@@ -36,6 +35,7 @@
     int OH, OW;
     int bn_T, bn_tc, bn_fps;
     int tiles_x, tiles_img;
+    int bn_slots, bn_slots_img;
     float x_th;
 };
 
@@ -88,10 +88,14 @@
 constexpr int BN_NT = 3;
 constexpr int BN_CMAX = 128;
 
-constexpr int RTH = 4, RTW = 32, RPITCH = RTW + 2, RCELLS = (RTH + 2) * RPITCH;
-
-template <int CO, bool F16, int ABL = 0, bool BNAP = false, bool RECT = false, bool SBF = false, bool XSP = false>
-__global__ __launch_bounds__(kThreads, 2) void k_conv_halo3(const float* __restrict__ x,
+constexpr int RTH = 4, RTW = 32, RPITCH = RTW + 2;
+
+constexpr int HBM_BIG = 2 * HBM_, HCELLS_BIG = 416, RTH_BIG = 2 * RTH;
+static_assert(HBM_BIG + 2 * 79 + 2 <= HCELLS_BIG, "halo of a 256-cell strip tile");
+
+template <int CO, bool F16, int ABL = 0, bool BNAP = false, bool RECT = false, bool SBF = false, bool XSP = false,
+          bool BIG = false>
+__global__ __launch_bounds__(kThreads, BIG && CO == 32 && RECT ? 3 : 2) void k_conv_halo3(const float* __restrict__ x,
                                                            const unsigned char* __restrict__ wimg,
                                                            float* __restrict__ y, HaloGeom g,
                                                            const float* __restrict__ addend,
@@ -99,19 +103,27 @@
                                                            const float* __restrict__ bn_y = nullptr,
                                                            const float* __restrict__ bn_coef = nullptr,
                                                            float* __restrict__ dy_out = nullptr) {
-    constexpr int WM = CO == 32 ? 4 : 2, WN = 4 / WM, TM = CO == 32 ? 1 : 2, TN = CO == 32 ? 1 : CO / 64;
+    constexpr int WM = (CO == 32 || BIG) ? 4 : 2, WN = 4 / WM, TM = (CO == 32 && !BIG) ? 1 : 2;
+    constexpr int TN = BIG ? CO / 32 : (CO == 32 ? 1 : CO / 64);
     static_assert(CO == 32 || CO == 64 || CO == 128, "channel tile");
     static_assert(!BNAP || CO >= 64, "the BatchNorm-apply variant covers the 64 / 128-channel tiles");
+    static_assert(!BIG || (CO <= 64 && F16 && !BNAP && !SBF && ABL == 0), "the 256-cell tile: 32 / 64-channel forward");
+    constexpr int TCELLS = BIG ? HBM_BIG : HBM_;
+    constexpr int TH = BIG ? RTH_BIG : RTH;
     constexpr int BTILE = (CO / 32) * 4096;
     constexpr int NDMA = (CO / 32) * 4 / 4;
     constexpr int ES = SBF ? 2 : 4;
     static_assert(!SBF || (!F16 && !BNAP && ABL == 0), "bf16 storage: bf16 MFMA, plain variant");
     static_assert(!XSP || (F16 && !BNAP && !SBF && ABL == 0), "spikes from potentials: the forward arithmetic, plain variant");
     constexpr int CF_BYTES = BNAP ? 3 * BN_NT * BN_CMAX * 4 : 0;
-    constexpr int HC = RECT ? (RCELLS + 31) / 32 * 32 : HCELLS;
+    constexpr int RC = (TH + 2) * RPITCH;
+    constexpr int HC = RECT ? (RC + 31) / 32 * 32 : (BIG ? HCELLS_BIG : HCELLS);
     constexpr int HP = HC * 64;
-    constexpr int RED_BYTES = (F16 || SBF) ? 4 * (CO == 128 ? 64 : 32) * 16 : 0;
-    __shared__ __attribute__((aligned(16))) unsigned char smem[2 * HP + 2 * BTILE + CF_BYTES + RED_BYTES];
+    constexpr int NP = HC / 32;
+    constexpr int RED_BYTES = (F16 || SBF) ? 4 * TN * 32 * 16 : 0;
+    constexpr int RED_OFF = BIG ? 2 * HP : 2 * HP + 2 * BTILE + CF_BYTES;
+    static_assert(!BIG || (RED_BYTES <= 2 * BTILE && 4 * 32 * (TN * 32 + 4) * 4 <= 2 * HP), "BIG: LDS regions");
+    __shared__ __attribute__((aligned(16))) unsigned char smem[2 * HP + 2 * BTILE + CF_BYTES + (BIG ? 0 : RED_BYTES)];
     unsigned char* Aimg = smem;
     unsigned char* Bimg = smem + 2 * HP;
     [[maybe_unused]] float* Cf = reinterpret_cast<float*>(smem + 2 * HP + 2 * BTILE);
@@ -138,7 +150,7 @@
     } else {
         grp = tile / g.tiles_per_group;
         kt = tile - grp * g.tiles_per_group;
-        c0 = kt * HBM_;
+        c0 = kt * TCELLS;
         const int R0g = c0 / g.PW;
         x0 = c0 - R0g * g.PW;
         const int ng = R0g / g.PH;
@@ -156,7 +168,7 @@
         xbytes > 0x7fffffffLL ? 0x7fffffff : (int)xbytes, 0x00020000);
     [[maybe_unused]] __amdgpu_buffer_rsrc_t rs_y = rs_x, rs_dy = rs_x;
     [[maybe_unused]] const int t_lo = BNAP ? nb / g.bn_fps : 0;
-    [[maybe_unused]] int cofs[NPASS];
+    [[maybe_unused]] int cofs[NP];
     [[maybe_unused]] unsigned imask = 0;
     [[maybe_unused]] unsigned vmask = 0;
     if constexpr (BNAP) {
@@ -171,19 +183,19 @@
             Cf[idx] = bn_coef[(int64_t)pl * g.bn_tc + (int64_t)t * g.Cin + c];
         }
     }
-    unsigned voff[NPASS];
-    int awr[NPASS];
-#pragma unroll
-    for (int p = 0; p < NPASS; ++p) {
+    unsigned voff[NP];
+    int awr[NP];
+#pragma unroll
+    for (int p = 0; p < NP; ++p) {
         const int cell = p * 32 + (tid >> 3);
         int xx, yy, n;
         bool ok;
         if constexpr (RECT) {
             const int rr = cell / RPITCH, cc = cell - rr * RPITCH;
-            yy = ty * RTH - 1 + rr;
+            yy = ty * TH - 1 + rr;
             xx = tx * RTW - 1 + cc;
             n = n0;
-            ok = cell < RCELLS && yy >= 0 && yy < g.H && xx >= 0 && xx < g.W;
+            ok = cell < RC && yy >= 0 && yy < g.H && xx >= 0 && xx < g.W;
         } else {
             const unsigned u = (unsigned)(x0 + cell + g.PW - 1);
             const unsigned dR = udiv_small(u, g.magic_pw);
@@ -239,10 +251,10 @@
     };
 
     using PReg = typename std::conditional<SBF, u32x2, f32x4>::type;
-    PReg pf[NPASS];
+    PReg pf[NP];
     auto store_halo = [&]() {
 #pragma unroll
-        for (int p = 0; p < NPASS; ++p) {
+        for (int p = 0; p < NP; ++p) {
             if constexpr (RECT)
                 if (p * 32 >= HC) continue;
             if constexpr (SBF) {
@@ -335,7 +347,7 @@
 
     dma_b(0, 0);
 #pragma unroll
-    for (int p = 0; p < NPASS; ++p) pf[p] = load_pass((int)voff[p]);
+    for (int p = 0; p < NP; ++p) pf[p] = load_pass((int)voff[p]);
     if constexpr (BNAP) {
         f32x4 py[NPASS];
 #pragma unroll
@@ -361,7 +373,12 @@
                 if (kk + 1 < nk) dma_b(kk + 1, cur ^ 1);
             __builtin_amdgcn_sched_barrier(0);
             if constexpr (!(ABL & 4)) {
-                if (BNAP || more) pf[tap] = load_pass(more ? (int)(voff[tap] + (unsigned)cbytes) : (int)0x80000000u);
+                if constexpr (BNAP) {
+                    pf[tap] = load_pass(more ? (int)(voff[tap] + (unsigned)cbytes) : (int)0x80000000u);
+                } else if (tap == 0 && more) {
+#pragma unroll
+                    for (int p = 0; p < NP; ++p) pf[p] = load_pass((int)(voff[p] + (unsigned)cbytes));
+                }
             }
             if constexpr (BNAP)
                 pfy[tap & 1] = __builtin_bit_cast(f32x4, __builtin_amdgcn_raw_buffer_load_b128(
@@ -400,7 +417,7 @@
         int xx, yy, n;
         bool ok;
         if constexpr (RECT) {
-            yy = ty * RTH + (m >> 5);
+            yy = ty * TH + (m >> 5);
             xx = tx * RTW + (m & 31);
             n = n0;
             ok = yy < g.H && xx < g.W && nch < g.Cout;
@@ -501,7 +518,7 @@
             ssum[q] += partner32(ssum[q]);
             qsum[q] += partner32(qsum[q]);
         }
-        double* red = reinterpret_cast<double*>(smem + 2 * HP + 2 * BTILE + CF_BYTES);
+        double* red = reinterpret_cast<double*>(smem + RED_OFF);
         if (lane >= 48 && lane < 48 + LPR) {
 #pragma unroll
             for (int q = 0; q < 4; ++q) {
@@ -510,7 +527,29 @@
             }
         }
         __syncthreads();
-        if (tid < CO) {
+        if constexpr (BIG) {
+            if (tid < 2 * CO) {
+                const int hf = tid / CO, cc = tid % CO;
+                int slot;
+                bool valid;
+                if constexpr (RECT) {
+                    const int ty4 = 2 * ty + hf;
+                    slot = (n0 - grp * g.G) * g.bn_slots_img + ty4 * g.tiles_x + tx;
+                    valid = ty4 * RTH < g.H;
+                } else {
+                    slot = 2 * kt + hf;
+                    valid = slot < g.bn_slots;
+                }
+                const double* s0 = red + ((2 * hf) * LPR * 4 + cc) * 2;
+                const double* s1 = red + ((2 * hf + 1) * LPR * 4 + cc) * 2;
+                const double s = s0[0] + s1[0], q2 = s0[1] + s1[1];
+                if (valid && n0c + cc < g.Cout) {
+                    double* dstp = g.bn_partial + snn_bn_partial_index(grp, slot, n0c + cc, g.bn_slots, g.Cout);
+                    dstp[0] = s;
+                    dstp[1] = q2;
+                }
+            }
+        } else if (tid < CO) {
             const int wn_ = tid / (TN * 32), cc = tid % (TN * 32);
             double s = 0.0, q2 = 0.0;
 #pragma unroll
@@ -529,22 +568,28 @@
 }
 
 constexpr int SPITCH = RTW + 1, SCELLS = (RTH + 1) * SPITCH;
-template <bool SBF = false, bool RECT = false>
-__global__ __launch_bounds__(kThreads, 2) void k_conv_s2dgrad3(const float* __restrict__ x,
+template <bool SBF = false, bool RECT = false, int NW = 4>
+__global__ __launch_bounds__(NW * 64, NW == 8 ? 4 : 2) void k_conv_s2dgrad3(const float* __restrict__ x,
                                                               const unsigned char* __restrict__ wimg,
                                                               float* __restrict__ y,
                                                               HaloGeom g, const float* __restrict__ addend,
                                                               const float* __restrict__ addend2) {
-    constexpr int CO = 64, TN = 2;
+    static_assert(NW == 4 || (NW == 8 && !SBF && !RECT), "eight waves: the fp32 strip form");
+    constexpr int CO = 64, WNS = NW / 4, TN = 2 / WNS;
     constexpr int ES = SBF ? 2 : 4;
     constexpr int BTILE = (CO / 32) * 4096;
-    constexpr int NDMA = (CO / 32) * 4 / 4;
-    __shared__ __attribute__((aligned(16))) unsigned char smem[2 * HPIECE + 2 * BTILE];
+    constexpr int NDMA = BTILE / (NW * 1024);
+    constexpr int CPP = NW * 8;
+    constexpr int NP = (HCELLS + CPP - 1) / CPP;
+    constexpr int HPS = NP * CPP * 64;
+    static_assert(NP <= 9, "one staging pass per tap at most");
+    __shared__ __attribute__((aligned(16))) unsigned char smem[2 * HPS + 2 * BTILE];
     unsigned char* Aimg = smem;
-    unsigned char* Bimg = smem + 2 * HPIECE;
+    unsigned char* Bimg = smem + 2 * HPS;
 
     const int tid = threadIdx.x, lane = tid & 63;
     const int wave = __builtin_amdgcn_readfirstlane(tid >> 6);
+    const int wr = wave / WNS, wn = wave % WNS;
     const int r = lane & 31, h = lane >> 5;
 
     const int bq = blockIdx.x >> 3;
@@ -574,11 +619,11 @@
     __amdgpu_buffer_rsrc_t rs_x = __builtin_amdgcn_make_buffer_rsrc(
         reinterpret_cast<char*>(const_cast<float*>(x)) + (int64_t)nb * ipix * g.ldx * ES, 0,
         xbytes > 0x7fffffffLL ? 0x7fffffff : (int)xbytes, 0x00020000);
-    unsigned voff[NPASS];
-    int awr[NPASS];
-#pragma unroll
-    for (int p = 0; p < NPASS; ++p) {
-        const int cell = p * 32 + (tid >> 3);
+    unsigned voff[NP];
+    int awr[NP];
+#pragma unroll
+    for (int p = 0; p < NP; ++p) {
+        const int cell = p * CPP + (tid >> 3);
         int xx, yy, n;
         bool ok;
         if constexpr (RECT) {
@@ -601,7 +646,7 @@
         voff[p] = ok ? (unsigned)((pix * g.ldx + quad * 4) * ES) : 0x80000000u;
         awr[p] = cell_slot_off(cell, quad >> 1) + (quad & 1) * 8;
     }
-    const int cellbase = RECT ? wave * SPITCH + r : wave * 32 + r;
+    const int cellbase = RECT ? wr * SPITCH + r : wr * 32 + r;
     const int nchunks = g.Cin >> 5;
     const int co_tiles = g.Cout >> 5;
     const unsigned char* wsrc = wimg + (int64_t)(n0c >> 5) * 4096 + lane * 16;
@@ -617,22 +662,22 @@
             unsigned keep;
             asm volatile("s_mov_b32 %0, m0\n\ts_mov_b32 m0, %2\n\ts_nop 0\n\tglobal_load_lds_dwordx4 %1, off\n\ts_mov_b32 m0, %0"
                          : "=&s"(keep)
-                         : "v"(src + q * 4096), "s"(__builtin_amdgcn_readfirstlane(dst + q * 4096))
+                         : "v"(src + q * NW * 1024), "s"(__builtin_amdgcn_readfirstlane(dst + q * NW * 1024))
                          : "memory");
         }
     };
     using PReg = typename std::conditional<SBF, u32x2, f32x4>::type;
-    PReg pf[NPASS];
+    PReg pf[NP];
     auto store_halo = [&]() {
 #pragma unroll
-        for (int p = 0; p < NPASS; ++p) {
+        for (int p = 0; p < NP; ++p) {
             if constexpr (SBF) {
                 *reinterpret_cast<u32x2*>(Aimg + awr[p]) = pf[p];
             } else {
                 u32x2 hi, lo;
                 split4<false>(pf[p], hi, lo);
                 *reinterpret_cast<u32x2*>(Aimg + awr[p]) = hi;
-                *reinterpret_cast<u32x2*>(Aimg + HPIECE + awr[p]) = lo;
+                *reinterpret_cast<u32x2*>(Aimg + HPS + awr[p]) = lo;
             }
         }
     };
@@ -654,10 +699,10 @@
             const int off = cell_slot_off(cellbase + tapoff, 2 * ks + h);
             const bf16x8 ah = *reinterpret_cast<const bf16x8*>(Aimg + off);
             bf16x8 al = ah;
-            if constexpr (!SBF) al = *reinterpret_cast<const bf16x8*>(Aimg + HPIECE + off);
+            if constexpr (!SBF) al = *reinterpret_cast<const bf16x8*>(Aimg + HPS + off);
 #pragma unroll
             for (int j = 0; j < TN; ++j) {
-                const int boff = j * 4096 + ks * 2048 + lane * 16;
+                const int boff = (wn * TN + j) * 4096 + ks * 2048 + lane * 16;
                 const bf16x8 bh = *reinterpret_cast<const bf16x8*>(Bb + boff);
                 if constexpr (!SBF) {
                     const bf16x8 bl = *reinterpret_cast<const bf16x8*>(Bb + boff + 1024);
@@ -671,7 +716,7 @@
 
     dma_b(0, 0);
 #pragma unroll
-    for (int p = 0; p < NPASS; ++p) pf[p] = load_pass((int)voff[p]);
+    for (int p = 0; p < NP; ++p) pf[p] = load_pass((int)voff[p]);
     store_halo();
     asm volatile("s_waitcnt vmcnt(0) lgkmcnt(0)\n\ts_barrier" ::: "memory");
 
@@ -686,7 +731,10 @@
             const int cur = kk & 1;
             if (kk + 1 < nk) dma_b(kk + 1, cur ^ 1);
             __builtin_amdgcn_sched_barrier(0);
-            if (more) pf[tap] = load_pass((int)(voff[tap] + (unsigned)cbytes));
+            if (tap == 0 && more) {
+#pragma unroll
+                for (int p = 0; p < NP; ++p) pf[p] = load_pass((int)(voff[p] + (unsigned)cbytes));
+            }
             __builtin_amdgcn_sched_barrier(0);
             const int kh = tap / 3, kw = tap - 3 * kh;
             const int ph = kh == 1 ? 0 : 1, pw = kw == 1 ? 0 : 1;
@@ -701,10 +749,11 @@
     }
 
     constexpr int EW = TN * 32 + 4, LPR = TN * 8, RPP = 64 / LPR;
+    static_assert(NW * 32 * EW * 4 <= 2 * HPS, "staging rows inside the halo image");
     float* stage = reinterpret_cast<float*>(smem) + wave * 32 * EW;
     const bool ovec = g.out_vec != 0;
     const int lrow = lane / LPR, c4 = (lane % LPR) * 4;
-    const int nch = n0c + c4;
+    const int nch = n0c + wn * TN * 32 + c4;
     const int cells_left = g.group_cells - c0;
 #pragma unroll
     for (int cls = 0; cls < 4; ++cls) {
@@ -718,11 +767,11 @@
 #pragma unroll
         for (int pass = 0; pass < 32 / RPP; ++pass) {
             const int row = pass * RPP + lrow;
-            const int m = wave * 32 + row;
+            const int m = wr * 32 + row;
             int aa, bb, n;
             bool inside;
             if constexpr (RECT) {
-                aa = ty * RTH + wave;
+                aa = ty * RTH + wr;
                 bb = tx * RTW + row;
                 n = n0;
                 inside = true;
@@ -824,6 +873,18 @@
     return tiles < 0x7fffffffLL ? 2 : 0;
 }
 static bool halo_shape_ok(int64_t N, int H, int W, int Cin, int Cout) { return halo_mode(N, H, W, Cin, Cout) != 0; }
+
+constexpr int64_t kBigMinBlocks = 512;
+static int halo_tile(int64_t N, int H, int W, int Cin, int Cout, int precision) {
+    const int mode = halo_mode(N, H, W, Cin, Cout);
+    if (mode == 0 || precision != SNN_PREC_FP16X3 || Cout % 128 == 0) return mode;
+    if (mode == 2 && Cout != 32) return mode;
+    if (snn_tuning_env("SNN_HALO_SMALL_TILE") || snn_tuning_env("SNN_HALO_ABL")) return mode;
+    const int64_t ntiles_n = Cout == 32 ? 1 : Cout / 64;
+    const int64_t tiles = mode == 1 ? snn_ceil_div(N * (int64_t)(H + 1) * (W + 1), HBM_BIG)
+                                    : N * snn_ceil_div(H, RTH_BIG) * snn_ceil_div(W, RTW);
+    return tiles * ntiles_n >= kBigMinBlocks ? mode + 2 : mode;
+}
 
 static bool s2dgrad_rect(int Wo) { return 128 + (Wo + 1) + 2 > HCELLS; }
 static bool s2dgrad_shape_ok(int64_t N, int H, int W, int Cin, int Ho, int Wo, int Cout) {
@@ -896,14 +957,21 @@
         hipLaunchKernelGGL((k_conv_s2dgrad3<true, false>), grid, dim3(kThreads), 0, (hipStream_t)stream, dy, wi, dx, g, addend, addend2);
     else if (rect)
         hipLaunchKernelGGL((k_conv_s2dgrad3<false, true>), grid, dim3(kThreads), 0, (hipStream_t)stream, dy, wi, dx, g, addend, addend2);
+    else if (snn_tuning_env("SNN_S2DGRAD_W4"))
+        hipLaunchKernelGGL((k_conv_s2dgrad3<false, false>), grid, dim3(kThreads), 0, (hipStream_t)stream, dy, wi, dx, g, addend, addend2);
     else
-        hipLaunchKernelGGL((k_conv_s2dgrad3<false, false>), grid, dim3(kThreads), 0, (hipStream_t)stream, dy, wi, dx, g, addend, addend2);
+        hipLaunchKernelGGL((k_conv_s2dgrad3<false, false, 8>), grid, dim3(2 * kThreads), 0, (hipStream_t)stream, dy, wi, dx, g,
+                           addend, addend2);
     SNN_CHECK_LAUNCH("snn_conv3x3_s2_dgrad");
     return 0;
 }
 
 extern "C" int snn_conv3x3_halo_supported(int64_t N, int H, int W, int Cin, int Cout) {
     return halo_shape_ok(N, H, W, Cin, Cout) ? 1 : 0;
+}
+
+extern "C" int snn_conv3x3_halo_kernel(int64_t N, int H, int W, int Cin, int Cout, int precision) {
+    return halo_tile(N, H, W, Cin, Cout, precision);
 }
 
 extern "C" int64_t snn_conv3x3_halo_bn_chunks(int frames_per_step, int H, int W) {
@@ -1012,21 +1080,25 @@
     HaloGeom g;
     g.ldx = ldx; g.ldy = ldy; g.ld_add = ld_addend; g.ld_add2 = ld_addend2;
     g.N = (int)N; g.H = H; g.W = W; g.Cin = Cin; g.Cout = Cout;
-    const bool rect = halo_mode(N, H, W, Cin, Cout) == 2;
+    const int kind = halo_tile(N, H, W, Cin, Cout, precision);
+    const bool rect = kind == 2 || kind == 4, big = kind >= 3;
     g.PW = W + 1; g.PH = H + 1;
     g.G = bn_partial ? frames_per_step : (int)N;
     g.tiles_x = (int)snn_ceil_div(W, RTW);
-    g.tiles_img = g.tiles_x * (int)snn_ceil_div(H, RTH);
+    g.tiles_img = g.tiles_x * (int)snn_ceil_div(H, big ? RTH_BIG : RTH);
+    g.bn_slots_img = g.tiles_x * (int)snn_ceil_div(H, RTH);
     int64_t tiles;
     if (rect) {
         g.group_cells = 0;
         g.tiles_per_group = g.G * g.tiles_img;
+        g.bn_slots = g.G * g.bn_slots_img;
         tiles = N * (int64_t)g.tiles_img;
         SNN_REQUIRE((int64_t)H * W * ldx * 4 < 0x7fffffffLL, "snn_conv3x3_halo: an image must span less than 2 GiB");
     } else {
         const int64_t group_cells = (int64_t)g.G * g.PH * g.PW;
         g.group_cells = (int)group_cells;
-        g.tiles_per_group = (int)snn_ceil_div(group_cells, HBM_);
+        g.tiles_per_group = (int)snn_ceil_div(group_cells, big ? HBM_BIG : HBM_);
+        g.bn_slots = (int)snn_ceil_div(group_cells, HBM_);
         tiles = (int64_t)(N / g.G) * g.tiles_per_group;
     }
     const int co_tile = Cout % 128 == 0 ? 128 : (Cout % 64 == 0 ? 64 : 32);
@@ -1041,13 +1113,20 @@
     g.OH = H; g.OW = W;
     g.bn_T = g.bn_tc = 0; g.bn_fps = 1;
     g.x_th = x_th;
-    if (bn_partial) bn_layout[0] = g.tiles_per_group;
+    if (bn_partial) bn_layout[0] = g.bn_slots;
     dim3 grid((unsigned)((int64_t)g.tiles_per_xcd * 8 * g.ntiles_n));
     const unsigned char* wi = static_cast<const unsigned char*>(w_image);
     const bool f16 = precision == SNN_PREC_FP16X3;
 #define SNN_HALO_LAUNCH(CO_, F16_)                                                                                   \
     do {                                                                                                              \
-        if (rect)                                                                                                     \
+        constexpr int CB_ = CO_ > 64 ? 64 : CO_;     \
+        if (kind == 3)                                                                                                \
+            hipLaunchKernelGGL((k_conv_halo3<CB_, true, 0, false, false, false, false, true>), grid, dim3(kThreads), 0, \
+                               (hipStream_t)stream, x, wi, y, g, addend, addend2, nullptr, nullptr, nullptr);          \
+        else if (kind == 4)                                                                                           \
+            hipLaunchKernelGGL((k_conv_halo3<32, true, 0, false, true, false, false, true>), grid, dim3(kThreads), 0,  \
+                               (hipStream_t)stream, x, wi, y, g, addend, addend2, nullptr, nullptr, nullptr);          \
+        else if (rect)                                                                                                \
             hipLaunchKernelGGL((k_conv_halo3<CO_, F16_, 0, false, true>), grid, dim3(kThreads), 0, (hipStream_t)stream, x, wi, \
                                y, g, addend, addend2, nullptr, nullptr, nullptr);                                     \
         else                                                                                                          \
@@ -1070,7 +1149,14 @@
     if (xsp) {
 #define SNN_HALO_LAUNCH_X(CO_)                                                                                       \
     do {                                                                                                              \
-        if (rect)                                                                                                     \
+        constexpr int CB_ = CO_ > 64 ? 64 : CO_;                           \
+        if (kind == 3)                                                                                                \
+            hipLaunchKernelGGL((k_conv_halo3<CB_, true, 0, false, false, false, true, true>), grid, dim3(kThreads), 0,  \
+                               (hipStream_t)stream, x, wi, y, g, addend, addend2, nullptr, nullptr, nullptr);          \
+        else if (kind == 4)                                                                                           \
+            hipLaunchKernelGGL((k_conv_halo3<32, true, 0, false, true, false, true, true>), grid, dim3(kThreads), 0,   \
+                               (hipStream_t)stream, x, wi, y, g, addend, addend2, nullptr, nullptr, nullptr);          \
+        else if (rect)                                                                                                \
             hipLaunchKernelGGL((k_conv_halo3<CO_, true, 0, false, true, false, true>), grid, dim3(kThreads), 0,          \
                                (hipStream_t)stream, x, wi, y, g, addend, addend2, nullptr, nullptr, nullptr);          \
         else                                                                                                          \
```
